# pmichels19/AdvancedGraphicsRayTracer

Measured on AMD Instinct MI355X. Metric: Mrays/s (primary+shadow) at 1080p, higher is better.
Workload: dtype f32

## Files before the change

advancedgraphicsraytracer_amd/__init__.py:

```python
import contextlib
import ctypes as C
import os

import numpy as np

PKG_DIR = os.path.dirname(os.path.abspath(__file__))
LIB_PATH = os.path.abspath(os.environ.get("RTAMD_LIB", os.path.join(PKG_DIR, "librtamd.so")))
DATA_DIR = os.path.join(PKG_DIR, "data")
HEADER = os.path.join(os.path.dirname(PKG_DIR), "include", "rt_amd.h")

ABI_VERSION = 4
RT_OK, RT_ERR_INVALID, RT_ERR_NO_DEVICE, RT_ERR_HIP, RT_ERR_IO, RT_ERR_UNSUPPORTED, RT_ERR_COMM = 0, -1, -2, -3, -4, -5, -6
RT_COMM_ID_BYTES = 128
MULTI_PIPELINED, MULTI_TIMING, MULTI_BALANCED = 1, 2, 4
SPHERE, PLANE, CUBE, QUAD, TRIANGLE = 0, 1, 2, 3, 4
DIFFUSE, MIRROR, DIELECTRIC, CHECKERBOARD, LIGHT, DSMIX, TEXTURE = 0, 1, 2, 3, 4, 5, 6
MODE_PATH = 0
MODE_WHITTED = 1
MODE_PACKET = 2
MODE_BVH_HEAT = 3
WALK_LANE, WALK_WAVE, WALK_AUTO = 0, 1, 2
WALK_CHECK_OFF, WALK_CHECK_COUNT, WALK_CHECK_VERIFY = 0, 1, 2
BVH_PLAIN, BVH_SBVH = 0, 1
DEFAULT_DEPTH = {MODE_PATH: 10, MODE_WHITTED: 20, MODE_PACKET: 10, MODE_BVH_HEAT: 1}
# ... 121 lines not shown
        "rt_bvh_visualize_host": ([vp, vp, vp, u32], C.c_int),
        "rt_scene_bvh_cost": ([vp, C.POINTER(BvhCost), vp], C.c_int),
        "rt_scene_update_triangles": ([vp, u32, u32, vp, vp], C.c_int),
        "rt_scene_update_triangles_host": ([vp, u32, u32, fp], C.c_int),
        "rt_scene_update_prims": ([vp, u32, u32, vp, vp, vp], C.c_int),
        "rt_scene_update_prims_host": ([vp, u32, u32, C.POINTER(Prim), fp], C.c_int),
        "rt_scene_transform_triangles": ([vp, C.POINTER(TriXform), u32, vp, vp], C.c_int),
        "rt_scene_update_triangles_async": ([vp, u32, u32, vp, vp, C.POINTER(C.c_uint64)], C.c_int),
        "rt_scene_update_prims_async": ([vp, u32, u32, vp, vp, vp, C.POINTER(C.c_uint64)], C.c_int),
        "rt_scene_transform_triangles_async": ([vp, C.POINTER(TriXform), u32, vp, vp, C.POINTER(C.c_uint64)], C.c_int),
        "rt_scene_update_sync": ([vp, C.POINTER(UpdateStatus)], C.c_int),
        "rt_scene_rebuild": ([vp, vp], C.c_int),
        "rt_scene_rebuild_stats": ([vp, C.POINTER(C.c_uint32)], C.c_int),
        "rt_scene_prepare_updates": ([vp, vp], C.c_int),
        "rt_scene_update_plan_info": ([vp, C.POINTER(C.c_uint32)], C.c_int),
        "rt_scene_copy_update_plan": ([vp, C.POINTER(u32), C.POINTER(u32), C.POINTER(u32)], C.c_int),
        "rt_bvh_refit_plan_host": ([vp, u32, C.POINTER(u32), u32, C.POINTER(C.POINTER(u32)), C.POINTER(C.POINTER(u32)),
                                    C.POINTER(C.POINTER(u32)), C.POINTER(u32)], C.c_int),
        "rt_scene_splice_triangles": ([vp, u32, u32, vp, u32, vp], C.c_int),
        "rt_scene_splice_triangles_host": ([vp, u32, u32, C.POINTER(Prim), u32], C.c_int),
        "rt_scene_splice_ranges": ([vp, C.POINTER(TriEdit), u32, vp, vp], C.c_int),
        "rt_scene_splice_ranges_host": ([vp, C.POINTER(TriEdit), u32, C.POINTER(Prim)], C.c_int),
        "rt_scene_compact_triangles": ([vp, vp, vp], C.c_int),
        "rt_scene_compact_triangles_host": ([vp, vp], C.c_int),
        "rt_scene_splice_prims": ([vp, C.POINTER(PrimEdit), u32, vp, vp, vp], C.c_int),
        "rt_scene_splice_prims_host": ([vp, C.POINTER(PrimEdit), u32, C.POINTER(Prim), fp], C.c_int),
        "rt_scene_compact_prims": ([vp, vp, vp], C.c_int),
        "rt_scene_compact_prims_host": ([vp, vp], C.c_int),
        "rt_scene_set_prim_materials": ([vp, u32, u32, vp, vp], C.c_int),
        "rt_scene_set_prim_materials_host": ([vp, u32, u32, C.POINTER(i32)], C.c_int),
        "rt_sbvh_build_host": ([C.POINTER(Prim), C.POINTER(C.c_float), u32, C.POINTER(vp), C.POINTER(C.POINTER(u32)),
                                C.POINTER(SceneInfo)], C.c_int),
        "rt_image_load": ([C.c_char_p, C.POINTER(C.POINTER(u32)), C.POINTER(u32), C.POINTER(u32)], C.c_int),
        "rt_scene_create": ([C.POINTER(SceneDesc), C.POINTER(vp)], C.c_int),
        "rt_scene_create_recipe": ([C.c_char_p, C.c_char_p, i32, C.POINTER(vp)], C.c_int),
        "rt_scene_create_recipe_ex": ([C.c_char_p, C.c_char_p, i32, i32, C.POINTER(vp)], C.c_int),
        "rt_scene_destroy": ([vp], C.c_int),
        "rt_scene_get_info": ([vp, C.POINTER(SceneInfo)], C.c_int),
        "rt_scene_set_camera_walk": ([vp, C.c_int], C.c_int),
        "rt_scene_copy_bvh": ([vp, vp, C.POINTER(u32)], C.c_int),
        "rt_intersect": ([vp, vp, vp, u32, vp], C.c_int),
        "rt_occluded": ([vp, vp, vp, u32, vp], C.c_int),
        "rt_intersect_host": ([vp, vp, vp, u32], C.c_int),
        "rt_occluded_host": ([vp, vp, vp, u32], C.c_int),
        "rt_intersect_packets": ([vp, vp, vp, u32, vp], C.c_int),
        "rt_intersect_packets_host": ([vp, vp, vp, u32], C.c_int),
        "rt_trace": ([vp, C.c_int, vp, vp, vp, u32, vp, vp, vp, u32, vp], C.c_int),
        "rt_trace_host": ([vp, C.c_int, vp, vp, vp, u32, vp, vp, vp, u32], C.c_int),
        "rt_comm_unique_id": ([vp], C.c_int),
        "rt_comm_create": ([vp, C.c_int, C.c_int, C.c_int, C.POINTER(vp)], C.c_int),
        "rt_comm_wrap": ([vp, C.c_int, C.POINTER(vp)], C.c_int),
        "rt_comm_info": ([vp, C.POINTER(C.c_int), C.POINTER(C.c_int)], C.c_int),
        "rt_comm_destroy": ([vp], C.c_int),
        "rt_render_frame_multi": ([vp, vp, C.POINTER(Camera), C.POINTER(FrameParams), vp, u32, vp], C.c_int),
        "rt_multi_flush": ([vp, vp, vp, vp], C.c_int),
        "rt_comm_timing": ([vp, C.POINTER(C.c_double), C.POINTER(C.c_double), C.POINTER(C.c_uint64)], C.c_int),
        "rt_comm_deal_info": ([vp, C.POINTER(C.c_int), C.POINTER(C.c_uint32), C.POINTER(C.c_uint32),
                               C.POINTER(C.c_uint64)], C.c_int),
        "rt_comm_deal_hash": ([vp, C.POINTER(C.c_uint64)], C.c_int),
        "rt_camera_default": ([u32, u32, C.POINTER(Camera)], C.c_int),
        "rt_renderer_create": ([vp, u32, u32, C.POINTER(vp)], C.c_int),
        "rt_renderer_destroy": ([vp], C.c_int),
        "rt_render_frame": ([vp, C.POINTER(Camera), C.POINTER(FrameParams), vp, vp], C.c_int),
        "rt_render_frame_host": ([vp, C.POINTER(Camera), C.POINTER(FrameParams), vp], C.c_int),
        "rt_render_gbuffer": ([vp, C.POINTER(Camera), C.POINTER(FrameParams), u32, u32, u32, u32, u32, C.POINTER(GBuffer), vp],
                              C.c_int),
        "rt_render_gbuffer_host": ([vp, C.POINTER(Camera), C.POINTER(FrameParams), u32, u32, u32, u32, u32, C.POINTER(GBuffer)],
                                   C.c_int),
        "rt_gbuffer_pixels": ([vp, C.POINTER(Camera), C.POINTER(FrameParams), u32, vp, u32, C.POINTER(GBuffer), vp], C.c_int),
        "rt_gbuffer_pixels_host": ([vp, C.POINTER(Camera), C.POINTER(FrameParams), u32, vp, u32, C.POINTER(GBuffer)], C.c_int),
        "rt_renderer_gbuffer_walk": ([vp, C.c_int, C.POINTER(C.c_int), C.POINTER(u32)], C.c_int),
        "rt_shard_capacity": ([u32, u32, u32, C.POINTER(u32)], C.c_int),
        "rt_render_shard": ([vp, C.POINTER(Camera), C.POINTER(FrameParams), u32, u32, vp, vp], C.c_int),
        "rt_assemble_shards": ([vp, vp, u32, vp, vp], C.c_int),
        "rt_tile_deal": ([u32, u32, C.POINTER(u32), u32, C.POINTER(u32), C.POINTER(u32)], C.c_int),
        "rt_render_shard_tiles": ([vp, C.POINTER(Camera), C.POINTER(FrameParams), C.POINTER(u32), u32, vp, vp], C.c_int),
        "rt_assemble_tiles": ([vp, vp, u32, C.POINTER(u32), C.POINTER(u32), u32, vp, vp], C.c_int),
        "rt_renderer_counters": ([vp, C.POINTER(Counters)], C.c_int),
        "rt_renderer_read_accumulator": ([vp, fp], C.c_int),
        "rt_renderer_overlap": ([vp, C.POINTER(C.c_int), fp], C.c_int),
        "rt_renderer_overlap_depth": ([vp, C.POINTER(C.c_int), fp], C.c_int),
        "rt_renderer_device_bytes": ([vp, C.POINTER(C.c_uint64), C.POINTER(C.c_uint32)], C.c_int),
        "rt_renderer_tile_costs": ([vp, C.POINTER(u32), u32, C.POINTER(u32)], C.c_int),
        "rt_renderer_tile_work": ([vp, C.POINTER(Camera), C.POINTER(FrameParams), C.POINTER(u32), u32, vp, vp], C.c_int),
        "rt_renderer_choices": ([vp, C.POINTER(C.c_int), C.POINTER(C.c_int), fp, fp], C.c_int),
        "rt_renderer_set_walk_check": ([vp, C.c_int], C.c_int),
        "rt_renderer_walk_stats": ([vp, C.POINTER(C.c_uint64)], C.c_int),
        "rt_renderer_stream": ([vp, C.POINTER(vp)], C.c_int),
        "rt_frame_kernel_name": ([vp, C.POINTER(FrameParams)], C.c_char_p),
        "rt_synchronize": ([vp], C.c_int),
    }
    for name, (args, res) in sigs.items():
        fn = getattr(L, name)
        fn.argtypes = args
        fn.restype = res
    if L.rt_abi_version() != ABI_VERSION:
        raise RTError(RT_ERR_INVALID, "librtamd.so ABI mismatch")
    _lib = L
    return L


def _check(rc):
    if rc != RT_OK:
        raise RTError(rc, lib().rt_last_error().decode(errors="replace"))
    return rc


def device_count():
    n = C.c_int(0)
    rc = lib().rt_device_count(C.byref(n))
    return n.value if rc == RT_OK else 0


def _fptr(a):
    return a.ctypes.data_as(C.POINTER(C.c_float))


def load_obj(path):
    return _take_mesh(lib().rt_obj_load, path)


def load_mesh(path):
    return _take_mesh(lib().rt_mesh_load, path)


def _take_mesh(fn, path):
    L = lib()
    vp, fp = C.POINTER(C.c_float)(), C.POINTER(C.c_int32)()
    nv, nt = C.c_uint32(), C.c_uint32()
    _check(fn(os.fsencode(path), C.byref(vp), C.byref(nv), C.byref(fp), C.byref(nt)))
    try:
        V = np.ctypeslib.as_array(vp, shape=(nv.value, 3)).copy() if nv.value else np.zeros((0, 3), np.float32)
        F = np.ctypeslib.as_array(fp, shape=(nt.value, 3)).copy() if nt.value else np.zeros((0, 3), np.int32)
    finally:
        L.rt_free(C.cast(vp, C.c_void_p))
        L.rt_free(C.cast(fp, C.c_void_p))
    return V, F


def save_mesh(path, verts, faces):
    V = np.ascontiguousarray(verts, np.float32)
    F = np.ascontiguousarray(faces, np.int32)
    _check(lib().rt_mesh_save(os.fsencode(path), _fptr(V), len(V), F.ctypes.data_as(C.POINTER(C.c_int32)), len(F)))


def mat4_translate(x, y, z):
    m = np.zeros(16, np.float32)
    _check(lib().rt_mat4_translate(x, y, z, _fptr(m)))
    return m


def mat4_scale(s):
    m = np.zeros(16, np.float32)
    _check(lib().rt_mat4_scale(s, _fptr(m)))
    return m


def mat4_rotate(axis, angle):
    m = np.zeros(16, np.float32)
    _check(lib().rt_mat4_rotate(axis, angle, _fptr(m)))
    return m


def mat4_mul(*ms):
    acc = np.ascontiguousarray(ms[0], np.float32).copy()
    for m in ms[1:]:
# ... 801 lines not shown
        if frame is None:
            self.frame += 1
        return out

    def render_shard_tiles(self, out, tiles, spp=1, depth=None, frame=None, reset=False, stream=None):
        torch = _torch()
        p = self.params(spp, depth, frame, reset)
        t = np.ascontiguousarray(tiles, np.uint32)
        s = stream if stream is not None else torch.cuda.current_stream(out.device).cuda_stream
        _check(self.L.rt_render_shard_tiles(self.h, C.byref(self.camera), C.byref(p), t.ctypes.data_as(C.POINTER(C.c_uint32)),
                                            len(t), C.c_void_p(out.data_ptr()), C.c_void_p(s)))
        if frame is None:
            self.frame += 1
        return out

    def assemble_tiles(self, gathered, stride_px, deal_tiles, deal_off, out, stream=None):
        torch = _torch()
        dt = np.ascontiguousarray(deal_tiles, np.uint32)
        do = np.ascontiguousarray(deal_off, np.uint32)
        s = stream if stream is not None else torch.cuda.current_stream(out.device).cuda_stream
        _check(self.L.rt_assemble_tiles(self.h, C.c_void_p(gathered.data_ptr()), stride_px,
                                        dt.ctypes.data_as(C.POINTER(C.c_uint32)), do.ctypes.data_as(C.POINTER(C.c_uint32)),
                                        len(do) - 1, C.c_void_p(out.data_ptr()), C.c_void_p(s)))
        return out

    def assemble(self, gathered, num_shards, out, stream=None):
        torch = _torch()
        s = stream if stream is not None else torch.cuda.current_stream(out.device).cuda_stream
        _check(self.L.rt_assemble_shards(self.h, C.c_void_p(gathered.data_ptr()), num_shards,
                                         C.c_void_p(out.data_ptr()), C.c_void_p(s)))
        return out

    def kernel_name(self, spp=1, depth=None):
        name = self.L.rt_frame_kernel_name(self.h, C.byref(self.params(spp, depth)))
        if name is None:
            raise RTError(-1, self.L.rt_last_error().decode())
        return name.decode()

    def counters(self):
        c = Counters()
        _check(self.L.rt_renderer_counters(self.h, C.byref(c)))
        return {n: int(getattr(c, n)) for n, _ in Counters._fields_}

    def overlap(self):
        st = C.c_int()
        ms = np.zeros(4, np.float32)
        _check(self.L.rt_renderer_overlap(self.h, C.byref(st), _fptr(ms)))
        return st.value, [round(float(x), 4) for x in ms]

    def overlap_depth(self):
        d = C.c_int()
        ms = np.zeros(8, np.float32)
        _check(self.L.rt_renderer_overlap_depth(self.h, C.byref(d), _fptr(ms)))
        return d.value, [round(float(x), 4) for x in ms]

    def device_bytes(self):
        b, n = C.c_uint64(), C.c_uint32()
        _check(self.L.rt_renderer_device_bytes(self.h, C.byref(b), C.byref(n)))
        return b.value, n.value

    def choices(self):
        w, sp = C.c_int(), C.c_int()
        wm, sm = np.zeros(4, np.float32), np.zeros(4, np.float32)
        _check(self.L.rt_renderer_choices(self.h, C.byref(w), C.byref(sp), _fptr(wm), _fptr(sm)))
        return {"walk": w.value, "split": sp.value, "walk_ms": [round(float(x), 4) for x in wm],
                "split_ms": [round(float(x), 4) for x in sm]}

    def set_walk_check(self, level):
        _check(self.L.rt_renderer_set_walk_check(self.h, level))

    def walk_stats(self):
        out = (C.c_uint64 * 4)()
        _check(self.L.rt_renderer_walk_stats(self.h, out))
        return {"walked": int(out[0]), "margin_boxes": int(out[1]), "retraced": int(out[2]), "verify_mismatch": int(out[3])}

    def tile_costs(self):
        n = C.c_uint32()
        _check(self.L.rt_renderer_tile_costs(self.h, None, 0, C.byref(n)))
        out = np.zeros(n.value, np.uint32)
        if n.value:
            _check(self.L.rt_renderer_tile_costs(self.h, out.ctypes.data_as(C.POINTER(C.c_uint32)), n.value, C.byref(n)))
        return out

    def tile_work(self, spp=1, depth=None, frame=None, pixels=False, stream=None):
        tx, ty = (self.width + 7) // 8, (self.height + 7) // 8
        work = np.zeros(tx * ty, np.uint32)
        p = self.params(spp, depth, frame)
        buf = None
        if pixels:
            torch = _torch()
            buf = torch.zeros(self.width * self.height * 8, dtype=torch.int32, device=f"cuda:{self.scene.device}")
        _check(self.L.rt_renderer_tile_work(self.h, C.byref(self.camera), C.byref(p),
                                            work.ctypes.data_as(C.POINTER(C.c_uint32)), len(work),
                                            None if buf is None else C.c_void_p(buf.data_ptr()),
                                            None if stream is None else C.c_void_p(stream)))
        if buf is None:
            return work
        return work, buf.view(-1, 8).cpu().numpy().view(np.uint32)

    def accumulator(self):
        acc = np.zeros((self.height * self.width, 4), np.float32)
        _check(self.L.rt_renderer_read_accumulator(self.h, _fptr(acc)))
        return acc
```

advancedgraphicsraytracer_amd/build.py:

```python
import os
import subprocess
import sys

PKG = os.path.dirname(os.path.abspath(__file__))
ROOT = os.path.dirname(PKG)
CSRC = os.path.join(PKG, "csrc")
LIB = os.path.join(PKG, "librtamd.so")
SOURCES = ["rt_host.cpp", "rt_device.hip", "rt_kern_core.hip", "rt_kern_ext.hip", "rt_multi.cpp", "rt_sbvh.cpp",
           "rt_refit.hip", "rt_build.hip", "rt_splice.hip", "rt_scene_pack.cpp", "rt_cost.hip", "rt_plan.hip", "rt_scene_edit.hip"]
HEADERS = ["rt_math.h", "rt_internal.h", "rt_libm.h", "rt_dev_types.h", "rt_variants.h", "rt_kernels.inc", "rt_refit.h", "rt_tune.h", "rt_sched.h",
           "rt_records.h", "rt_update.h", "rt_build.h", "rt_splice.h", "rt_cost.h", "rt_plan.h", "rt_scene.h", os.path.join("..", "..", "include", "rt_amd.h")]

HIPCC = os.environ.get("HIPCC", "/opt/rocm/bin/hipcc")
LIBS = ["-lz", "-ldl"]
FLAGS = ["--offload-arch=gfx950", "-O3", "-std=c++17", "-ffp-contract=off", "-fno-slp-vectorize", "-fPIC",
         "-shared",
         "-Wall", "-Wno-unused-function"]


def _source_hash():
    import hashlib
    h = hashlib.sha256()
    for f in [os.path.join(CSRC, x) for x in SOURCES + HEADERS] + [os.path.abspath(__file__)]:
        with open(f, "rb") as fh:
            h.update(os.path.basename(f).encode() + b"\0" + fh.read())
    h.update(" ".join(FLAGS + LIBS).encode())
    return h.hexdigest()


STAMP = LIB + ".srchash"


def _stale():
    if not os.path.exists(LIB) or not os.path.exists(STAMP):
        return True
    with open(STAMP) as f:
        return f.read().strip() != _source_hash()


def build(force=False, verbose=False):
    if not force and not _stale():
        return LIB
    objdir = os.path.join(PKG, "_obj")
    os.makedirs(objdir, exist_ok=True)
    compile_flags = [f for f in FLAGS if f != "-shared"]
    procs = []
    objs = []
    for f in SOURCES:
        obj = os.path.join(objdir, os.path.splitext(f)[0] + ".o")
        lang = ["-x", "hip"]
        cmd = [HIPCC] + compile_flags + lang + ["-c", os.path.join(CSRC, f), "-o", obj]
        if verbose:
            print(" ".join(cmd), file=sys.stderr)
        procs.append((f, subprocess.Popen(cmd, stdout=subprocess.PIPE, stderr=subprocess.PIPE, text=True)))
        objs.append(obj)
    for f, p in procs:
        out, err = p.communicate()
        if p.returncode != 0:
            raise RuntimeError(f"hipcc failed on {f} ({p.returncode}):\n{out}\n{err}")
    cmd = [HIPCC, "--offload-arch=gfx950", "-fPIC", "-shared", "--hip-link", "-o", LIB + ".tmp"] + objs + LIBS
    if verbose:
        print(" ".join(cmd), file=sys.stderr)
    r = subprocess.run(cmd, capture_output=True, text=True)
    if r.returncode != 0:
        raise RuntimeError(f"link failed ({r.returncode}):\n{r.stdout}\n{r.stderr}")
    os.replace(LIB + ".tmp", LIB)
    with open(STAMP, "w") as f:
        f.write(_source_hash() + "\n")
    return LIB


if __name__ == "__main__":
    print(build(force="--force" in sys.argv, verbose=True))
```

advancedgraphicsraytracer_amd/csrc/rt_dev_types.h:

```cpp
#pragma once
#include <hip/hip_runtime.h>

#include <cstdint>

#include "../../include/rt_amd.h"
#include "rt_variants.h"

namespace rt {

enum : uint32_t { T_TRI = 4, T_SPH = 0, T_PLANE = 1, T_CUBE = 2, T_QUAD = 3 };
enum : int { F_DIFFUSE = 0, F_SPECULAR = 1, F_MIX = 2, F_DIELECTRIC = 3, F_LIGHT = 4 };

struct DevMaterial {
    int kind, flag;
    float c0[3], c1[3];
    float ior, diffuse, specular;
    uint32_t tex_off, tex_w, tex_h;
    uint32_t pad_[2];
};
static_assert(sizeof(DevMaterial) == 64, "DevMaterial is read as four float4");

struct SceneView {
    const float4 *__restrict__ nodes;
    const float4 *__restrict__ prims;
    const float4 *__restrict__ shade;
    const DevMaterial *__restrict__ mats;
    const uint32_t *__restrict__ sky;
    const float4 *__restrict__ xprims;
    const uint32_t *__restrict__ tex;
    uint32_t sky_w, sky_h;
    int sky_const;
    float sky_rgb[3];
    float light_M[12];
    float light_c[3];
    float light_r, light_r2, light_invr;
    int light_mat;
    int light_quad;
    float light_qsize, light_area;
    float light_N[3];
    uint32_t root_word;
    int bounds_finite;
    uint32_t stack_entries;
    int wave_primary;
    int walk_check;
    float walk_margin;
    const float4 *__restrict__ quads;
    uint32_t quad_root;
    int quad_lanes;
    unsigned long long *walk_stats;
};

constexpr uint32_t kCounterSlots = 1024;

constexpr size_t kLdsLaunchMax = 65536;
constexpr size_t kWorkCounterBytes = 8u * 256u * sizeof(uint32_t);

struct FrameArgs {
    float cam_pos[3], cam_tl[3], cam_tr[3], cam_bl[3];
    float lens, rw, rh;
    uint32_t W, H, spp, depth, frame, reset;
    uint32_t shard, nshards, tiles_x, ntiles_local;
    const uint32_t *tile_map;
    uint32_t nchunks, nunits;
    float4 *samples;
    int packed_out;
    const uint32_t *order;
    uint32_t part_shift;
    uint32_t *tile_cost;
    float4 *acc;
    uint32_t *out;
    const uint32_t *fwd_src;
    uint32_t *fwd_dst;
    unsigned long long *counters;
};

struct FrameLaunch {
    FrameVariant v;
    dim3 grid;
    size_t lds_bytes;
    hipStream_t stream;
};

constexpr uint32_t kQueueSegs = 16;

struct PathArgs {
    uint32_t s0, batch_spp, npaths, level;
    uint32_t seg_cap;
    int dynamic;
    uint32_t *qhead;
    uint32_t drain_level, drain_below;
    float4 *state;
    float4 *rec;
    float4 *result;
    uint32_t *queue_in, *queue_out;
    uint32_t *qcount;
    float4 *sum;
    uint32_t *tile_cost;
};

struct TraceArgs {
    const rt_ray *rays;
    uint32_t *seeds;
    const uint8_t *flags;
    float *radiance;
    rt_hit *hits;
    unsigned long long *counts;
    uint32_t n, depth;
};

struct GBufferArgs {
    rt_ray *ray;
    rt_hit *hit;
    rt_gnormal *normal;
    rt_galbedo *albedo;
    uint32_t sample;
    uint32_t x0, y0, w, h;
    uint32_t tx0, ty0, ntx, ntiles;
    const uint32_t *pixels;
    uint32_t n;
};

struct Launchers {
    void (*frame)(const SceneView &S, const FrameArgs &F, const FrameLaunch &L);
    void (*work)(const SceneView &S, const FrameArgs &F, const FrameLaunch &L, uint32_t *tile_work, uint32_t *pixel_work);
    void (*intersect)(const SceneView &S, const rt_ray *rays, rt_hit *hits, uint32_t n, size_t lds, hipStream_t st);
    void (*occluded)(const SceneView &S, const rt_ray *rays, uint8_t *out, uint32_t n, size_t lds, hipStream_t st);
    void (*intersect_packet)(const SceneView &S, const rt_ray *rays, rt_hit *hits, uint32_t n, hipStream_t st);
    int (*pt_level)(const SceneView &S, const FrameArgs &F, const PathArgs &P, bool tex, size_t lds, uint32_t num_cus,
                    hipStream_t st);
    void (*pt_lanes)(const SceneView &S, const FrameArgs &F, const PathArgs &P, bool tex, size_t lds, uint32_t num_cus,
                     hipStream_t st);
    void (*pt_finish)(const FrameArgs &F, const PathArgs &P, bool last, hipStream_t st);
    void (*trace)(const SceneView &S, const TraceArgs &A, const FrameVariant &v, size_t lds, hipStream_t st);
    void (*gbuffer)(const SceneView &S, const FrameArgs &F, const GBufferArgs &G, const GBufferVariant &v, size_t lds,
                    hipStream_t st);
};
namespace kext {
const Launchers &launchers();
}
namespace kcore {
const Launchers &launchers();
void launch_heat(const SceneView &S, const FrameArgs &F, size_t lds, hipStream_t st);
void launch_visualize(const SceneView &S, const rt_ray *rays, uint32_t *counts, uint32_t n, size_t lds, hipStream_t st);
}
void launch_assemble(const uint32_t *gathered, uint32_t cap, uint32_t nshards, const uint32_t *where, uint32_t tiles_x,
                     uint32_t ntiles, uint32_t W, uint32_t H, uint32_t *out, hipStream_t st, uint32_t first = 0);

}
```

advancedgraphicsraytracer_amd/csrc/rt_device.hip:

```cpp
#include <hip/hip_runtime.h>

#include <algorithm>
#include <cmath>
#include <cstdlib>
#include <cstring>
#include <mutex>
#include <string>
#include <vector>

#include "rt_cost.h"
#include "rt_dev_types.h"
#include "rt_internal.h"
#include "rt_records.h"
#include "rt_refit.h"
#include "rt_scene.h"
#include "rt_sched.h"
#include "rt_tune.h"

using namespace rt;

constexpr int kPsMaxDepth = 8;
constexpr int kPtMaxSlots = 8;
inline int hw_queues() {
    const char *e = std::getenv("GPU_MAX_HW_QUEUES");
    const int v = e ? std::atoi(e) : 0;
    return v > 0 ? v : 4;
}

template <int N>
struct ResultRing {
    DevBuf buf[N];
    hipEvent_t fin[N] = {};
    bool fin_set[N] = {};

    int event(int b) {
        if (!fin[b]) HIP_TRY(hipEventCreateWithFlags(&fin[b], hipEventDisableTiming | hipEventReleaseToDevice));
        return RT_OK;
    }
    int ensure(int b, size_t bytes) {
        if (bytes <= buf[b].bytes) return RT_OK;
        fin_set[b] = false;
        return buf[b].grow(bytes, Wait::kDevice);
    }
    int drop_from(int k) {
        for (int b = k; b < N; ++b) {
            if (int rc = buf[b].release(); rc != RT_OK) return rc;
            fin_set[b] = false;
        }
        return RT_OK;
    }
    float4 *at(int b) const { return buf[b].template as<float4>(); }
};

struct rt_renderer {
    rt_scene *scene = nullptr;
    int device = 0;
    uint32_t W = 0, H = 0;
    float4 *d_acc = nullptr;
    unsigned long long *d_counters = nullptr;
    uint32_t *d_rgb = nullptr;
    uint64_t primary = 0, frames = 0;
    hipStream_t stream = nullptr;
    DevBuf d_order, d_cost;
    std::vector<uint32_t> host_cost;
    bool tail_bound = false;
    uint32_t order_n = 0;
    uint64_t order_key = 0;
    int order_state = 0;
    uint32_t order_split = 0;
    uint32_t order_parts = 2;
    TimedGroups walk_tg, split_tg, ps_tg;
    hipEvent_t tune_ev[4][16] = {};
    float walk_ms[4] = {}, split_ms[4] = {}, ps_ms[8] = {};
    int wave = -1;
    bool use_split = false;
    int ps_use = -1;
    uint64_t walk_key = 0;
    hipEvent_t stall_ev = nullptr;
    bool stall_armed = false;
    int walk_check = RT_WALK_CHECK_OFF;
    DevBuf d_pt[kPtMaxSlots];
    ResultRing<kPtMaxSlots + 1> pt_res;
    float4 *d_sum = nullptr;
    hipStream_t pt_stream[kPsMaxDepth] = {};
    int nstreams = 0;

    hipEvent_t pt_lv[kPsMaxDepth] = {};
    int pt_slot = 0, pt_parity = 0;
    uint32_t pt_nslots = 0;
    size_t pt_need = 0;
    bool pt_serial_last = false;
    uint64_t ps_last = 0;
    uint32_t ps_prev = 0;
    hipEvent_t ps_join = nullptr;
    hipEvent_t cost_ev = nullptr;
    ResultRing<kPsMaxDepth + 1> ps_res;
    uint32_t ps_count = 0;
    uint64_t gate_key = 0;
    int gate_state = 0;
    uint32_t gate_frames = 0;
    DevBuf d_samples;
    std::vector<uint32_t> map_host;
    int held_kind = 0;
    uint32_t held_shard = 0, held_nshards = 1;
    std::vector<uint32_t> held_list;
    uint64_t map_gen = 0, held_gen = 0;
    DevBuf d_work;
    DevBuf d_map;
    uint64_t map_hash = 0;
    DevBuf d_where;
    uint64_t where_hash = 0;
    TileGrid grid() const { return tile_grid(W, H); }
};

template <class R, class Fn>
void each_buffer(R &r, Fn f) {
    for (auto &b : r.d_pt) f(b);
    for (auto &b : r.pt_res.buf) f(b);
    for (auto &b : r.ps_res.buf) f(b);
    for (auto *b : {&r.d_samples, &r.d_order, &r.d_cost, &r.d_map, &r.d_work, &r.d_where}) f(*b);
}

namespace {

enum { kWalk, kSplit, kOverlap, kGate };

void free_scene(rt_scene *s) {
    if (!s) return;
    (void)hipSetDevice(s->device);
    (void)hipDeviceSynchronize();
    void *ptrs[] = {s->d_nodes, s->d_prims, s->d_shade, s->d_mats, s->d_sky, s->d_xprims, s->d_tex, s->d_scratch, s->d_quads, s->d_cost};
    for (void *p : ptrs)
        if (p) (void)hipFree(p);
    free_refit(s->refit);
    if (s->stream) (void)hipStreamDestroy(s->stream);
    delete s;
}

int ensure_device(int device) {
    int count = 0;
    if (hipGetDeviceCount(&count) != hipSuccess || count == 0)
        return fail(RT_ERR_NO_DEVICE, "no HIP device visible: the MI355X path has no CPU fallback");
    if (device < 0 || device >= count) return fail(RT_ERR_INVALID, "device index out of range");
    HIP_TRY(hipSetDevice(device));
    return RT_OK;
}

#ifndef RT_PT_QUADS_DEFAULT
#define RT_PT_QUADS_DEFAULT 0
#endif
int pack_options_from_env(PackOptions &o) {
    if (const char *e = std::getenv("RT_BVH")) {
        if (std::strcmp(e, "sbvh") != 0 && std::strcmp(e, "plain") != 0)
            return fail(RT_ERR_INVALID, std::string("RT_BVH must be 'plain' or 'sbvh', not '") + e + "'");
        o.bvh_kind = std::strcmp(e, "sbvh") == 0 ? RT_BVH_SBVH : RT_BVH_PLAIN;
    }
    if (const char *e = std::getenv("RT_WALK_MARGIN")) o.walk_margin = std::ldexp(1.0f, std::max(-40, std::min(-1, std::atoi(e))));
    if (const char *e = std::getenv("RT_WALK_STICKY")) o.sliver_lim = std::atoi(e) >= 0 ? 0.0 : std::ldexp(1.0, std::atoi(e));
    if (const char *e = std::getenv("RT_WALK_STICKY_SPHERES")) o.sticky_spheres = std::atoi(e) != 0;
    o.quads = RT_PT_QUADS_DEFAULT != 0;
    if (const char *e = std::getenv("RT_PT_QUADS")) o.quads = std::atoi(e) != 0;
    return RT_OK;
}

}

void rt::scene_tree_fields(rt_scene *s, uint32_t root_word, bool nested, bool bounds_finite) {
    s->stack_depth = pick_stack(s->bvh.depth);
    s->walk_fits = stack_admits_walk(s->stack_depth);
    s->nested = nested;
    SceneView &v = s->view;
    v.nodes = (const float4 *)s->d_nodes;
    v.prims = (const float4 *)s->d_prims;
    v.root_word = root_word;
    v.stack_entries = s->stack_depth;
    v.bounds_finite = bounds_finite ? 1 : 0;
    s->xcd_order = (size_t)s->bvh.nodes_used * 32u + (size_t)s->num_prims * 48u > (4u << 20);
    if (const char *e = std::getenv("RT_XCD_ORDER")) s->xcd_order = std::atoi(e) != 0;
    if (s->walk != RT_WALK_LANE && !(s->nested && s->walk_fits)) s->walk = RT_WALK_LANE;
}

namespace {

void scene_knobs_from_env(rt_scene *s) {
    if (const char *e = std::getenv("RT_PT_WAVEFRONT")) s->pt_wavefront = std::atoi(e) != 0;
    if (const char *e = std::getenv("RT_PT_DYNAMIC")) s->pt_dynamic = std::atoi(e) != 0;
    if (const char *e = std::getenv("RT_PT_LANES")) s->pt_lanes = std::atoi(e) != 0;
    if (const char *e = std::getenv("RT_PT_DRAIN_LEVEL")) s->pt_drain_level = (uint32_t)std::max(1, std::atoi(e));
    if (const char *e = std::getenv("RT_PT_DRAIN_ROUNDS")) s->pt_drain_rounds = std::max(0.0, std::atof(e));
    if (const char *e = std::getenv("RT_PT_DRAIN_SMALL")) s->pt_drain_small = (uint32_t)std::max(0, std::atoi(e));
    if (const char *e = std::getenv("RT_PT_SMALL_ROUNDS")) s->pt_small_rounds = std::max(0.0, std::atof(e));
    if (const char *e = std::getenv("RT_PT_SMALL_DRAIN_ROUNDS")) s->pt_small_drain_rounds = std::max(0.0, std::atof(e));
    if (const char *e = std::getenv("RT_TILE_ORDER")) s->tile_order = std::atoi(e) != 0;
    if (const char *e = std::getenv("RT_SPLIT_UNITS")) s->split_units = (uint32_t)std::max(0, std::atoi(e));
    if (const char *e = std::getenv("RT_FRAME_WAVES")) {
        const int w = std::atoi(e);
        s->frame_waves = w == 7 || w == 8 ? w : 0;
    }
    if (const char *e = std::getenv("RT_SPLIT_HEAVY")) s->heavy_split = std::max(-1, std::atoi(e));
    if (const char *e = std::getenv("RT_SPLIT_PARTS")) {
        const int k = std::atoi(e);
        s->split_parts = k >= 8 ? 8u : k >= 4 ? 4u : 2u;
    }
    if (const char *e = std::getenv("RT_PT_PIPELINE")) s->pt_pipeline = std::atoi(e) != 0;
    if (const char *e = std::getenv("RT_PT_SLOTS")) s->pt_slots = (uint32_t)std::max(2, std::min((int)kPtMaxSlots, std::atoi(e)));
    if (const char *e = std::getenv("RT_PS_PIPELINE")) s->ps_pipeline = std::max(-1, std::min(1, std::atoi(e)));
    if (const char *e = std::getenv("RT_PS_BUFFERS")) s->ps_buffers = (uint32_t)std::max(2, std::min(kPsMaxDepth + 1, std::atoi(e)));
    if (const char *e = std::getenv("RT_PS_DEPTH")) s->ps_depth = (uint32_t)std::max(2, std::min(kPsMaxDepth, std::atoi(e)));
    if (const char *e = std::getenv("RT_TUNE_DELAY_MS")) s->tune_delay_ms = (float)std::max(0.0, std::atof(e));
    if (const char *e = std::getenv("RT_PT_MEM_MB"))
        s->pt_mem_bytes = std::max<uint64_t>(1, std::strtoull(e, nullptr, 10)) << 20;
    const bool wave_ok = !s->has_cubes && s->nested && s->walk_fits;
    s->walk = wave_ok ? RT_WALK_AUTO : RT_WALK_LANE;
    if (const char *e = std::getenv("RT_WAVE_PRIMARY")) s->walk = std::atoi(e) != 0 && wave_ok ? RT_WALK_WAVE : RT_WALK_LANE;
}

int scene_create(const rt_scene_desc *d, rt_scene **out) {
    if (!d || !out) return fail(RT_ERR_INVALID, "rt_scene_create: empty or null description");
    *out = nullptr;
    PackOptions o;
    int rc = pack_options_from_env(o);
    if (rc != RT_OK) return rc;
    ScenePack p;
    if ((rc = pack_scene(d, o, p)) != RT_OK) return rc;
    if ((rc = ensure_device(d->device)) != RT_OK) return rc;

    rt_scene *s = new rt_scene();
    s->device = d->device;
    s->num_prims = d->num_prims;
    s->num_materials = d->num_materials;
    s->ext = p.ext;
    s->ext_fixed = p.ext_fixed;
    s->has_cubes = p.has_cubes;
    s->refit.boxes_finite = p.boxes_finite;
    s->quads = s->quad_lanes = p.has_quads;
    s->refit.sliver_lim = o.sliver_lim;
    s->refit.sticky_spheres = o.sticky_spheres;
    rc = upload(&s->d_nodes, p.nodes);
    if (rc == RT_OK) rc = upload(&s->d_prims, p.prims);
    if (rc == RT_OK) rc = upload(&s->d_shade, p.shade);
    if (rc == RT_OK) rc = upload(&s->d_mats, p.mats);
    if (rc == RT_OK) rc = upload(&s->d_sky, p.sky);
    if (rc == RT_OK) rc = upload(&s->d_xprims, p.xprims);
    if (rc == RT_OK) rc = upload(&s->d_tex, p.texels);
    if (rc == RT_OK && s->quads) rc = upload(&s->d_quads, p.quads);
    if (rc == RT_OK && hipStreamCreateWithFlags(&s->stream, hipStreamNonBlocking) != hipSuccess)
        rc = fail(RT_ERR_HIP, "hipStreamCreate failed");
    if (rc != RT_OK) { free_scene(s); return rc; }
    s->bvh = std::move(p.bvh);
    s->refit.pinfo = std::move(p.pinfo);
    s->refit.pbox = std::move(p.pbox);
    s->refit.pcen = std::move(p.pcen);

    SceneView &v = s->view;
    v = p.view;
    scene_tree_fields(s, p.view.root_word, p.nested, p.view.bounds_finite != 0);
    v.shade = (const float4 *)s->d_shade;
    v.mats = (const DevMaterial *)s->d_mats;
    v.sky = (const uint32_t *)s->d_sky;
    v.xprims = (const float4 *)s->d_xprims;
    v.tex = (const uint32_t *)s->d_tex;
    v.quads = s->quads ? (const float4 *)s->d_quads : nullptr;
    {
        hipDeviceProp_t prop;
        if (hipGetDeviceProperties(&prop, s->device) == hipSuccess && prop.multiProcessorCount > 0)
            s->num_cus = (uint32_t)prop.multiProcessorCount;
    }
    scene_knobs_from_env(s);
    *out = s;
    return RT_OK;
}

size_t stack_bytes(const rt_scene *s) { return (size_t)s->stack_depth * 256u * sizeof(uint32_t); }
size_t walk_bytes(const rt_scene *s, const SceneView &v) {
    return v.wave_primary ? (size_t)s->stack_depth * 4u * sizeof(uint32_t) : 0u;
}
// ... 154 lines not shown
        }
        if (!pipe) {
            const bool last = s0 + P.batch_spp >= F.spp;
            K.pt_finish(F, P, last, st);
        }
    }
    if (pipe) {
        for (int k = 0; k < (int)r->pt_nslots; ++k)
            if (used[k]) {
                HIP_TRY(hipEventRecord(r->pt_lv[k], r->pt_stream[k]));
                HIP_TRY(hipStreamWaitEvent(st, r->pt_lv[k], 0));
            }
        PathArgs P{};
        P.result = r->pt_res.at(par);
        P.sum = r->d_sum;
        P.s0 = 0;
        P.batch_spp = F.spp;
        K.pt_finish(F, P, true, st);
        HIP_TRY(hipEventRecord(r->pt_res.fin[par], st));
        r->pt_res.fin_set[par] = true;
    }
    HIP_TRY(hipGetLastError());
    return RT_OK;
}

int ensure_order(rt_renderer *r, uint64_t key, uint32_t n) {
    if (key == r->order_key && n == r->order_n) return RT_OK;
    r->order_key = key;
    r->order_state = 0;
    r->host_cost.clear();
    if (n != r->order_n) {
        HIP_TRY(hipDeviceSynchronize());
        r->order_n = 0;
        int rc = r->d_order.release();
        if (rc == RT_OK) rc = r->d_cost.release();
        if (rc == RT_OK) rc = r->d_order.grow(order_capacity(n) * sizeof(uint32_t));
        if (rc == RT_OK) rc = r->d_cost.grow(2u * (size_t)n * sizeof(uint32_t));
        if (rc != RT_OK) return rc;
        r->order_n = n;
    }
    return RT_OK;
}

struct FramePlan {
    uint64_t key = 0;
    bool gate_open = false, stalled = false;
    TimedFrame walk, split, ps;
    int cost_map = -1;
    bool walk_pending = false;
    uint32_t depth = 0, buf = 0, lane = 0;
};

int tile_order_step(rt_renderer *r, FrameArgs &F, bool split_ok, FramePlan &P) {
    const uint32_t n = F.ntiles_local;
    const int walk_phase = P.cost_map >= 0 ? P.cost_map : P.walk.decide ? 2 : P.walk_pending ? 3 : -1;
    if (P.key != r->order_key || n != r->order_n) {
        r->tail_bound = false;
        r->ps_tg.stop();
        r->ps_use = -1;
    }
    if (int rc = ensure_order(r, P.key, n); rc != RT_OK) return rc;
    uint32_t *const d_cost = r->d_cost.as<uint32_t>(), *const d_order = r->d_order.as<uint32_t>();
    int use = -1;
    if (walk_phase == 3) {
    } else if (r->order_state == 0) {
        if (walk_phase == 0 || walk_phase == 1) F.tile_cost = d_cost + (size_t)walk_phase * n;
        else if (walk_phase == 2) use = r->wave;
        else { F.tile_cost = d_cost; r->order_state = 1; }
    } else if (r->order_state == 1) {
        use = 0;
    }
    if (use >= 0) {
        HIP_TRY(hipDeviceSynchronize());
        std::vector<uint32_t> cost(n);
        HIP_TRY(hipMemcpy(cost.data(), d_cost + (size_t)use * n, n * sizeof(uint32_t), hipMemcpyDeviceToHost));
        r->host_cost = cost;
        r->tail_bound = tail_bound(cost, r->scene->num_cus, F.nchunks);
        const uint32_t k = split_count(n, r->scene->heavy_split, split_ok), parts = r->scene->split_parts;
        const TileWhere where{F.tiles_x, F.shard, F.nshards, F.tile_map ? r->map_host.data() : nullptr};
        const std::vector<uint32_t> ent = build_tile_order(cost, k, parts, r->scene->xcd_order && split_ok, where);
        HIP_TRY(hipMemcpy(d_order, ent.data(), ent.size() * sizeof(uint32_t), hipMemcpyHostToDevice));
        r->order_split = k;
        r->order_parts = parts;
        r->order_state = 2;
        r->use_split = k > 0 && r->scene->heavy_split > 0;
        r->split_tg.stop();
        if (k > 0 && r->scene->heavy_split < 0) {
            start_two_way(r->split_tg, false);
            if (int rc = ensure_events(r->tune_ev[kSplit], 8); rc != RT_OK) return rc;
        }
    }
    if (r->order_state == 2) {
        P.split = r->split_tg.next(P.gate_open, P.stalled);
        if (P.split.decide) {
            if (int rc = group_times(r->tune_ev[kSplit], 4, r->split_ms); rc != RT_OK) return rc;
            r->use_split = tuned_alternative(r->split_ms);
        }
        const bool split = P.split.group >= 0 ? alternative_group(P.split) : r->use_split;
        F.order = split ? d_order + n : d_order;
        F.nunits = order_units(F.ntiles_local, F.nchunks, split, r->order_split, r->order_parts);
        F.part_shift = part_shift(r->order_parts);
    }
    return RT_OK;
}

uint64_t param_key(const rt_renderer *r, const FrameArgs &F, const rt_camera *cam, const rt_frame_params *p) {
    uint64_t key = fnv1a(cam, sizeof(*cam));
    key = fnv1a(&p->width, sizeof(uint32_t) * 4, key);
    key = fnv1a(&p->mode, sizeof(uint32_t), key);
    key = fnv1a(&F.shard, sizeof(uint32_t) * 2, key);
    if (F.tile_map) key = fnv1a(&r->map_hash, sizeof(r->map_hash), key);
    return key;
}

int tune_gate(rt_renderer *r, uint64_t key, hipStream_t st, bool &open) {
    const float delay = r->scene->tune_delay_ms;
    if (key != r->gate_key) {
        r->gate_key = key;
        r->gate_state = 0;
    }
    if (delay <= 0.0f) r->gate_state = 3;
    if (r->gate_state == 3) { open = true; return RT_OK; }
    open = false;
    if (int rc = ensure_events(r->tune_ev[kGate], 2); rc != RT_OK) return rc;
    if (r->gate_state == 0) {
        HIP_TRY(hipEventRecord(r->tune_ev[kGate][0], st));
        r->gate_state = 1;
        r->gate_frames = 0;
    } else if (r->gate_state == 1) {
        if (++r->gate_frames % 8 == 0) {
            HIP_TRY(hipEventRecord(r->tune_ev[kGate][1], st));
            r->gate_state = 2;
        }
    } else if (hipEventQuery(r->tune_ev[kGate][1]) == hipSuccess) {
        float ms = 0.0f;
        HIP_TRY(hipEventElapsedTime(&ms, r->tune_ev[kGate][0], r->tune_ev[kGate][1]));
        r->gate_state = ms >= delay ? 3 : 1;
        open = r->gate_state == 3;
    }
    return RT_OK;
}

int frame_args(rt_renderer *r, const rt_camera *cam, const rt_frame_params *p, uint32_t shard, uint32_t nshards,
               const uint32_t *tiles, uint32_t ntiles_map, FrameArgs &F) {
    if (p->width != r->W || p->height != r->H)
        return fail(RT_ERR_INVALID, "frame size differs from the renderer's accumulator");
    if (p->spp == 0) return fail(RT_ERR_INVALID, "spp must be >= 1");
    if (p->mode > RT_MODE_BVH_HEAT) return fail(RT_ERR_INVALID, "unknown integrator mode");
    if (nshards == 0 || shard >= nshards) return fail(RT_ERR_INVALID, "bad shard index");
    HIP_TRY(hipSetDevice(r->scene->device));
    F = FrameArgs{};
    for (int i = 0; i < 3; ++i) {
        F.cam_pos[i] = cam->pos[i]; F.cam_tl[i] = cam->top_left[i];
        F.cam_tr[i] = cam->top_right[i]; F.cam_bl[i] = cam->bottom_left[i];
    }
    F.lens = cam->lens_radius;
    F.rw = 1.0f / (float)r->W;
    F.rh = 1.0f / (float)r->H;
    F.W = r->W; F.H = r->H; F.spp = p->spp; F.depth = p->depth; F.frame = p->frame; F.reset = p->reset ? 1 : 0;
    const TileGrid g = r->grid();
    F.shard = shard; F.nshards = nshards; F.tiles_x = g.tiles_x;
    F.ntiles_local = local_tiles(g.ntiles, shard, nshards);
    if (tiles) {
        int rc = set_tile_map(r, tiles, ntiles_map, g.ntiles);
        if (rc != RT_OK) return rc;
        F.ntiles_local = ntiles_map;
        F.tile_map = r->d_map.as<uint32_t>();
    }
    F.acc = r->d_acc;
    F.counters = r->d_counters;
    F.nchunks = 1;
    F.nunits = F.ntiles_local;
    return RT_OK;
}

int work_frame(rt_renderer *r, const rt_camera *cam, const rt_frame_params *p, uint32_t shard, uint32_t nshards,
               const uint32_t *tiles, uint32_t ntiles_map, std::vector<uint32_t> &work, uint32_t *pixel_work,
               hipStream_t st) {
    if (!r || !cam || !p) return fail(RT_ERR_INVALID, "work frame: null argument");
    if (p->mode != RT_MODE_PATH) return fail(RT_ERR_UNSUPPORTED, "work frame: RT_MODE_PATH frames only");
    if (p->depth > 32) return fail(RT_ERR_UNSUPPORTED, "Trace depth above 32");
    if (stack_bytes(r->scene) + kWorkCounterBytes > kLdsLaunchMax)
        return fail(RT_ERR_UNSUPPORTED, "work frame: this tree's stacks leave no LDS for the counters");
    FrameArgs F;
    int rc = frame_args(r, cam, p, shard, nshards, tiles, ntiles_map, F);
// ... 138 lines not shown
        P.batch_spp = F.spp;
        P.result = F.samples;
        launchers(s).pt_finish(F, P, true, st);
        HIP_TRY(hipGetLastError());
        if (o.depth > 0) {
            HIP_TRY(hipEventRecord(r->ps_res.fin[o.buf], st));
            r->ps_res.fin_set[o.buf] = true;
        }
    }
    if (o.ps.ev_after >= 0) HIP_TRY(hipEventRecord(r->tune_ev[kOverlap][o.ps.ev_after], st));
    if (r->walk_tg.running() || r->split_tg.active() || r->ps_tg.active()) {
        if (!r->stall_ev) HIP_TRY(hipEventCreateWithFlags(&r->stall_ev, hipEventDisableTiming));
        HIP_TRY(hipEventRecord(r->stall_ev, st));
        r->stall_armed = true;
    }
    return RT_OK;
}

int launch_render(rt_renderer *r, const rt_camera *cam, const rt_frame_params *p, uint32_t shard, uint32_t nshards,
                  uint32_t *out, int packed, void *stream, const uint32_t *tiles = nullptr, uint32_t ntiles_map = 0,
                  const uint32_t *fwd_src = nullptr, uint32_t *fwd_dst = nullptr) {
    if (!r || !cam || !p || !out) return fail(RT_ERR_INVALID, "rt_render: null argument");
    if ((fwd_src || fwd_dst) && (packed || !fwd_src || !fwd_dst)) return fail(RT_ERR_INVALID, "rt_render: bad forward");
    rt_scene *s = r->scene;
    FrameArgs F;
    if (int rc = frame_args(r, cam, p, shard, nshards, tiles, ntiles_map, F); rc != RT_OK) return rc;
    if (tiles) {
        if (r->held_kind != 3 || r->held_gen != r->map_gen) {
            r->held_list = r->map_host;
            r->held_gen = r->map_gen;
        }
        r->held_kind = 3;
    } else {
        r->held_kind = nshards == 1 ? 1 : 2;
        r->held_shard = shard;
        r->held_nshards = nshards;
    }
    F.packed_out = packed;
    F.out = out;
    F.fwd_src = fwd_src;
    F.fwd_dst = fwd_dst;
    if (F.ntiles_local == 0) return RT_OK;
    hipStream_t st = (hipStream_t)stream;
    if (int rc = after_updates(s, st); rc != RT_OK) return rc;
    if (p->mode == RT_MODE_BVH_HEAT) {
        F.depth = s->bvh.depth;
        kcore::launch_heat(s->view, F, stack_bytes(s), st);
        HIP_TRY(hipGetLastError());
        r->primary += frame_pixels(r, F) * p->spp;
        r->frames += 1;
        return RT_OK;
    }
    if (p->depth > 32) return fail(RT_ERR_UNSUPPORTED, "Trace depth above 32");
    const int mode = (int)p->mode;
    const bool wavefront = mode == RT_MODE_PATH && p->depth >= 2 && s->pt_wavefront;
    if (int rc = sample_split(r, p->spp, mode != RT_MODE_PACKET && !wavefront, F); rc != RT_OK) return rc;
    if (wavefront) {
        if (int rc = wavefront_frame(r, F, cam, p, st); rc != RT_OK) return rc;
        r->primary += frame_pixels(r, F) * p->spp;
        r->frames += 1;
        return RT_OK;
    }
    FrameLaunch L{{}, dim3((F.nunits + 3) / 4), stack_bytes(s), st};
    SceneView view = s->view;
    view.walk_stats = r->d_counters;
    view.walk_check = r->walk_check;
    FramePlan P;
    P.key = param_key(r, F, cam, p);
    if (int rc = tune_gate(r, P.key, st, P.gate_open); rc != RT_OK) return rc;
    P.stalled = r->stall_armed && hipEventQuery(r->stall_ev) == hipSuccess;
    r->stall_armed = false;
    const bool ps_kernel = primary_shadow(mode, p->depth);
    if (int rc = walk_step(r, ps_kernel && !s->ext, view, P); rc != RT_OK) return rc;
    if (s->tile_order) {
        if (int rc = tile_order_step(r, F, ps_kernel && F.nchunks <= 1, P); rc != RT_OK) return rc;
        L.grid = dim3((F.nunits + 3) / 4);
    }
    const uint64_t ps_bytes = (uint64_t)p->spp * F.ntiles_local * 64u * 16u;
    const bool ps_ok = s->ps_pipeline != 0 && ps_kernel && !r->split_tg.active() && !F.tile_cost && !P.walk_pending &&
                       ps_bytes <= (2ull << 30);
    if (int rc = overlap_step(r, F, L, ps_ok, ps_bytes, st, P); rc != RT_OK) return rc;
    if (L.stream != st)
        if (int rc = after_updates(s, L.stream); rc != RT_OK) return rc;
    L.lds_bytes = stack_bytes(s) + walk_bytes(s, view);
    L.v = frame_variant({mode, p->depth, !view.sky_const, s->frame_waves, F.nchunks, F.spp, F.nunits, s->num_cus,
                         P.depth > 0, view.wave_primary, view.walk_check});
    if (int rc = submit_frame(r, view, F, L, P, st); rc != RT_OK) return rc;
    r->primary += frame_pixels(r, F) * p->spp;
    r->frames += 1;
    return RT_OK;
}

template <class Launch>
int ray_call(rt_scene *s, const void *rays, void *out, uint32_t n, void *stream, const char *null_text, Launch launch) {
    if (!s || (n && (!rays || !out))) return fail(RT_ERR_INVALID, null_text);
    if (n == 0) return RT_OK;
    HIP_TRY(hipSetDevice(s->device));
    hipStream_t st = (hipStream_t)stream;
    if (int rc = after_updates(s, st); rc != RT_OK) return rc;
    launch(st);
    HIP_TRY(hipGetLastError());
    return RT_OK;
}

int gbuffer_arguments(const std::string &name, const void *r, const rt_camera *cam, const rt_frame_params *p, uint32_t sample,
                      const rt_gbuffer *out) {
    if (!r || !cam || !p || !out) return fail(RT_ERR_INVALID, name + ": null argument");
    if (!out->ray && !out->hit && !out->normal && !out->albedo) return fail(RT_ERR_INVALID, name + ": no plane asked for");
    if (sample >= std::max(1u, p->spp)) return fail(RT_ERR_INVALID, name + ": sample outside the frame's samples per pixel");
    return RT_OK;
}
int gbuffer_rectangle(const std::string &name, const rt_frame_params *p, uint32_t x0, uint32_t y0, uint32_t w, uint32_t h) {
    if (!w || !h) return fail(RT_ERR_INVALID, name + ": empty rectangle");
    if (x0 >= p->width || w > p->width - x0 || y0 >= p->height || h > p->height - y0)
        return fail(RT_ERR_INVALID, name + ": the rectangle leaves the frame");
    return RT_OK;
}
int gbuffer_device() {
    static const bool have = [] {
        int count = 0;
        return hipGetDeviceCount(&count) == hipSuccess && count > 0;
    }();
    return have ? RT_OK : fail(RT_ERR_NO_DEVICE, "no HIP device visible: the MI355X path has no CPU fallback");
}
SceneView gbuffer_view(const rt_renderer *r, bool pixels, size_t &lds) {
    const rt_scene *s = r->scene;
    SceneView view = s->view;
    view.wave_primary = gbuffer_wave_walk({pixels, s->walk, r->wave, s->ext, s->has_cubes, s->nested, s->walk_fits}) ? 1 : 0;
    view.walk_check = RT_WALK_CHECK_OFF;
    view.walk_stats = nullptr;
    lds = stack_bytes(s) + walk_bytes(s, view);
    return view;
}
int gbuffer_launch(rt_renderer *r, const rt_camera *cam, const rt_frame_params *p, GBufferArgs &G, bool pixels, hipStream_t st) {
    if (int rc = gbuffer_device(); rc != RT_OK) return rc;
    rt_frame_params q = *p;
    q.spp = std::max(1u, p->spp);
    q.mode = RT_MODE_PATH;
    FrameArgs F;
    if (int rc = frame_args(r, cam, &q, 0, 1, nullptr, 0, F); rc != RT_OK) return rc;
    F.acc = nullptr;
    F.counters = nullptr;
    if (pixels && G.n == 0) return RT_OK;
    rt_scene *s = r->scene;
    if (int rc = after_updates(s, st); rc != RT_OK) return rc;
    size_t lds = 0;
    const SceneView view = gbuffer_view(r, pixels, lds);
    launchers(s).gbuffer(view, F, G, gbuffer_variant(pixels, !view.sky_const), lds, st);
    HIP_TRY(hipGetLastError());
    return RT_OK;
}
GBufferArgs gbuffer_planes(const rt_gbuffer *out, uint32_t sample) {
    GBufferArgs G{};
    G.ray = out->ray; G.hit = out->hit; G.normal = out->normal; G.albedo = out->albedo;
    G.sample = sample;
    return G;
}
template <class Run>
int gbuffer_staged(rt_renderer *r, const rt_frame_params *p, const uint32_t *list, size_t count, const rt_gbuffer *out, Run run) {
    if (int rc = gbuffer_device(); rc != RT_OK) return rc;
    if (p->width != r->W || p->height != r->H) return fail(RT_ERR_INVALID, "frame size differs from the renderer's accumulator");
    if (count == 0) return RT_OK;
    rt_scene *s = r->scene;
    HIP_TRY(hipSetDevice(s->device));
    auto up = [](size_t b) { return (b + 255) & ~(size_t)255; };
    void *const host[4] = {out->ray, out->hit, out->normal, out->albedo};
// ... 255 lines not shown
             : kind == CALL_VISUALIZE ? rt_bvh_visualize(s, d_rays, (uint32_t *)d_out, n, s->stream)
                                    : rt_intersect(s, d_rays, (rt_hit *)d_out, n, s->stream);
    if (rc != RT_OK) return rc;
    HIP_TRY(hipMemcpyAsync(out, d_out, out_elem * n, hipMemcpyDeviceToHost, s->stream));
    HIP_TRY(hipStreamSynchronize(s->stream));
    return RT_OK;
}

int rt_intersect_host(rt_scene *s, const rt_ray *rays, rt_hit *hits, uint32_t n) {
    return staged_call(s, rays, hits, sizeof(rt_hit), n, CALL_INTERSECT);
}
int rt_occluded_host(rt_scene *s, const rt_ray *rays, uint8_t *out, uint32_t n) {
    return staged_call(s, rays, out, 1, n, CALL_OCCLUDED);
}
int rt_intersect_packets_host(rt_scene *s, const rt_ray *rays, rt_hit *hits, uint32_t n) {
    return staged_call(s, rays, hits, sizeof(rt_hit), n, CALL_PACKETS);
}

int rt_bvh_visualize(rt_scene *s, const rt_ray *rays, uint32_t *counts, uint32_t n, void *stream) {
    return ray_call(s, rays, counts, n, stream, "rt_bvh_visualize: null argument",
                    [&](hipStream_t st) { kcore::launch_visualize(s->view, rays, counts, n, stack_bytes(s), st); });
}
int rt_bvh_visualize_host(rt_scene *s, const rt_ray *rays, uint32_t *counts, uint32_t n) {
    return staged_call(s, rays, counts, 2 * sizeof(uint32_t), n, CALL_VISUALIZE);
}

int rt_scene_bvh_cost(rt_scene *s, rt_bvh_cost *out, void *stream) {
    if (!s || !out) return fail(RT_ERR_INVALID, "rt_scene_bvh_cost: null argument");
    if (int frc = fold_updates(s); frc != RT_OK) return frc;
    if (!s->view.bounds_finite) return fail(RT_ERR_UNSUPPORTED, "rt_scene_bvh_cost: a node bound is NaN or infinite");
    HIP_TRY(hipSetDevice(s->device));
    rt_bvh_cost c{};
    const int rc = device_bvh_cost(s->d_nodes, s->bvh.nodes_used, &s->d_cost, (hipStream_t)stream, &c);
    if (rc == RT_OK) *out = c;
    return rc;
}

int rt_renderer_create(rt_scene *s, uint32_t W, uint32_t H, rt_renderer **out) {
    if (!s || !out || !W || !H) return fail(RT_ERR_INVALID, "rt_renderer_create: bad argument");
    if ((uint64_t)W * H >= (1ull << 31)) return fail(RT_ERR_UNSUPPORTED, "frame too large");
    HIP_TRY(hipSetDevice(s->device));
    rt_renderer *r = new rt_renderer();
    r->scene = s;
    r->device = s->device;
    r->W = W; r->H = H;
    start_two_way(r->walk_tg, true);
    hipError_t e = hipStreamCreateWithFlags(&r->stream, hipStreamNonBlocking);
    if (e == hipSuccess) e = hipMalloc(&r->d_acc, sizeof(float4) * (size_t)W * H);
    if (e == hipSuccess) e = hipMemsetAsync(r->d_acc, 0, sizeof(float4) * (size_t)W * H, r->stream);
    if (e == hipSuccess) e = hipMalloc(&r->d_counters, kCounterSlots * 8 * sizeof(unsigned long long));
    if (e == hipSuccess) e = hipMemsetAsync(r->d_counters, 0, kCounterSlots * 8 * sizeof(unsigned long long), r->stream);
    if (e == hipSuccess) e = hipStreamSynchronize(r->stream);
    if (e != hipSuccess) {
        if (r->d_acc) (void)hipFree(r->d_acc);
        if (r->d_counters) (void)hipFree(r->d_counters);
        if (r->stream) (void)hipStreamDestroy(r->stream);
        delete r;
        return fail(RT_ERR_HIP, std::string("rt_renderer_create: ") + hipGetErrorString(e));
    }
    *out = r;
    return RT_OK;
}

int rt_renderer_destroy(rt_renderer *r) {
    if (!r) return RT_OK;
    (void)hipSetDevice(r->device);
    (void)hipDeviceSynchronize();
    (void)hipFree(r->d_acc);
    (void)hipFree(r->d_counters);
    if (r->d_rgb) (void)hipFree(r->d_rgb);
    if (r->d_sum) (void)hipFree(r->d_sum);
    each_buffer(*r, [](DevBuf &b) { (void)b.release(); });
    for (int k = 0; k < kPsMaxDepth; ++k) {
        if (r->pt_stream[k]) (void)hipStreamDestroy(r->pt_stream[k]);
        if (r->pt_lv[k]) (void)hipEventDestroy(r->pt_lv[k]);
    }
    for (auto &row : r->tune_ev)
        for (auto &e : row)
            if (e) (void)hipEventDestroy(e);
    for (hipEvent_t e : r->pt_res.fin)
        if (e) (void)hipEventDestroy(e);
    for (hipEvent_t e : r->ps_res.fin)
        if (e) (void)hipEventDestroy(e);
    for (hipEvent_t e : {r->ps_join, r->cost_ev, r->stall_ev})
        if (e) (void)hipEventDestroy(e);
    (void)hipStreamDestroy(r->stream);
    delete r;
    return RT_OK;
}

int rt_render_frame(rt_renderer *r, const rt_camera *cam, const rt_frame_params *p, uint32_t *rgb8, void *stream) {
    return launch_render(r, cam, p, 0, 1, rgb8, 0, stream);
}

int rt_render_frame_host(rt_renderer *r, const rt_camera *cam, const rt_frame_params *p, uint32_t *rgb8) {
    if (!r || !rgb8) return fail(RT_ERR_INVALID, "rt_render_frame_host: null argument");
    HIP_TRY(hipSetDevice(r->scene->device));
    if (!r->d_rgb) HIP_TRY(hipMalloc(&r->d_rgb, sizeof(uint32_t) * (size_t)r->W * r->H));
    int rc = launch_render(r, cam, p, 0, 1, r->d_rgb, 0, r->stream);
    if (rc != RT_OK) return rc;
    HIP_TRY(hipMemcpyAsync(rgb8, r->d_rgb, sizeof(uint32_t) * (size_t)r->W * r->H, hipMemcpyDeviceToHost, r->stream));
    HIP_TRY(hipStreamSynchronize(r->stream));
    return RT_OK;
}

int rt_render_gbuffer(rt_renderer *r, const rt_camera *cam, const rt_frame_params *p, uint32_t sample, uint32_t x0, uint32_t y0,
                      uint32_t w, uint32_t h, const rt_gbuffer *out, void *stream) {
    const char *name = "rt_render_gbuffer";
    if (int rc = gbuffer_arguments(name, r, cam, p, sample, out); rc != RT_OK) return rc;
    if (int rc = gbuffer_rectangle(name, p, x0, y0, w, h); rc != RT_OK) return rc;
    GBufferArgs G = gbuffer_planes(out, sample);
    G.x0 = x0; G.y0 = y0; G.w = w; G.h = h;
    G.tx0 = x0 / 8u; G.ty0 = y0 / 8u;
    G.ntx = (x0 + w + 7u) / 8u - G.tx0;
    G.ntiles = G.ntx * ((y0 + h + 7u) / 8u - G.ty0);
    return gbuffer_launch(r, cam, p, G, false, (hipStream_t)stream);
}

int rt_render_gbuffer_host(rt_renderer *r, const rt_camera *cam, const rt_frame_params *p, uint32_t sample, uint32_t x0,
                           uint32_t y0, uint32_t w, uint32_t h, const rt_gbuffer *out) {
    const char *name = "rt_render_gbuffer_host";
    if (int rc = gbuffer_arguments(name, r, cam, p, sample, out); rc != RT_OK) return rc;
    if (int rc = gbuffer_rectangle(name, p, x0, y0, w, h); rc != RT_OK) return rc;
    return gbuffer_staged(r, p, nullptr, (size_t)w * h, out, [&](const uint32_t *, const rt_gbuffer *dev, hipStream_t st) {
        return rt_render_gbuffer(r, cam, p, sample, x0, y0, w, h, dev, st);
    });
}

int rt_gbuffer_pixels(rt_renderer *r, const rt_camera *cam, const rt_frame_params *p, uint32_t sample, const uint32_t *pixels,
                      uint32_t n, const rt_gbuffer *out, void *stream) {
    const char *name = "rt_gbuffer_pixels";
    if (int rc = gbuffer_arguments(name, r, cam, p, sample, out); rc != RT_OK) return rc;
    if (n && !pixels) return fail(RT_ERR_INVALID, std::string(name) + ": null pixel list");
    GBufferArgs G = gbuffer_planes(out, sample);
    G.pixels = pixels;
    G.n = n;
    return gbuffer_launch(r, cam, p, G, true, (hipStream_t)stream);
}

int rt_gbuffer_pixels_host(rt_renderer *r, const rt_camera *cam, const rt_frame_params *p, uint32_t sample,
                           const uint32_t *pixels, uint32_t n, const rt_gbuffer *out) {
    const char *name = "rt_gbuffer_pixels_host";
    if (int rc = gbuffer_arguments(name, r, cam, p, sample, out); rc != RT_OK) return rc;
    if (n && !pixels) return fail(RT_ERR_INVALID, std::string(name) + ": null pixel list");
    for (uint32_t i = 0; i < n; ++i)
        if (pixels[i] >= (uint64_t)p->width * p->height)
            return fail(RT_ERR_INVALID, std::string(name) + ": pixel " + std::to_string(i) + " lies outside the frame");
    return gbuffer_staged(r, p, pixels, n, out, [&](const uint32_t *list, const rt_gbuffer *dev, hipStream_t st) {
        return rt_gbuffer_pixels(r, cam, p, sample, list, n, dev, st);
    });
}

int rt_renderer_gbuffer_walk(const rt_renderer *r, int pixels, int *wave_walk, uint32_t *lds_bytes) {
    if (!r || !wave_walk) return fail(RT_ERR_INVALID, "rt_renderer_gbuffer_walk: null argument");
    size_t lds = 0;
    *wave_walk = gbuffer_view(r, pixels != 0, lds).wave_primary;
    if (lds_bytes) *lds_bytes = (uint32_t)lds;
    return RT_OK;
}

int rt_shard_capacity(uint32_t W, uint32_t H, uint32_t nshards, uint32_t *pixels) {
    if (!pixels || !nshards || !W || !H) return fail(RT_ERR_INVALID, "rt_shard_capacity: bad argument");
    *pixels = local_tiles(tile_grid(W, H).ntiles, 0, nshards) * 64u;
    return RT_OK;
}

int rt_render_shard(rt_renderer *r, const rt_camera *cam, const rt_frame_params *p, uint32_t shard, uint32_t nshards,
// ... 79 lines not shown
    std::vector<unsigned long long> c((size_t)kCounterSlots * 8);
    HIP_TRY(hipMemcpy(c.data(), r->d_counters, c.size() * sizeof(unsigned long long), hipMemcpyDeviceToHost));
    for (int i = 0; i < 4; ++i) out[i] = 0;
    for (uint32_t k = 0; k < kCounterSlots; ++k) {
        out[0] += c[(size_t)k * 8 + 4];
        out[1] += c[(size_t)k * 8 + 2];
        out[2] += c[(size_t)k * 8 + 3];
        out[3] += c[(size_t)k * 8 + 5];
    }
    return RT_OK;
}

int rt_renderer_overlap(const rt_renderer *r, int *state, float ms[4]) {
    if (!r || !state) return fail(RT_ERR_INVALID, "rt_renderer_overlap: null argument");
    int depth = 0;
    float all[8];
    rt_renderer_overlap_depth(r, &depth, all);
    *state = depth < 0 ? -1 : (depth > 1 ? 1 : 0);
    if (ms) {
        const int n = r->ps_tg.groups == 8 ? 8 : 4;
        const int g[4] = {0, 1, n - 2, n - 1};
        for (int k = 0; k < 4; ++k) ms[k] = all[g[k]];
    }
    return RT_OK;
}

int rt_renderer_choices(const rt_renderer *r, int *walk, int *split, float walk_ms[4], float split_ms[4]) {
    if (!r || !walk || !split) return fail(RT_ERR_INVALID, "rt_renderer_choices: null argument");
    const rt_scene *s = r->scene;
    const bool split_set = r->order_state == 2 && !r->split_tg.active();
    *walk = s->walk == RT_WALK_WAVE ? 1 : s->walk == RT_WALK_LANE ? 0 : r->wave;
    *split = split_set ? (r->use_split ? 1 : 0) : -1;
    for (int g = 0; g < 4; ++g) {
        if (walk_ms) walk_ms[g] = (r->wave >= 0 && s->walk == RT_WALK_AUTO) ? r->walk_ms[g] : 0.0f;
        if (split_ms) split_ms[g] = split_set ? r->split_ms[g] : 0.0f;
    }
    return RT_OK;
}

int rt_renderer_overlap_depth(const rt_renderer *r, int *depth, float ms[8]) {
    if (!r || !depth) return fail(RT_ERR_INVALID, "rt_renderer_overlap_depth: null argument");
    const int32_t mode = r->scene->ps_pipeline;
    const bool decided = mode < 0 && r->ps_use >= 0;
    if (mode == 0) *depth = 1;
    else if (mode == 1) *depth = (int)r->scene->ps_depth;
    else *depth = decided ? (r->ps_use ? r->ps_use : 1) : -1;
    if (ms)
        for (int g = 0; g < 8; ++g) ms[g] = (decided && g < r->ps_tg.groups) ? r->ps_ms[g] : 0.0f;
    return RT_OK;
}

int rt_renderer_device_bytes(const rt_renderer *r, uint64_t *bytes, uint32_t *ps_buffers) {
    if (!r || !bytes) return fail(RT_ERR_INVALID, "rt_renderer_device_bytes: null argument");
    const uint64_t pix = (uint64_t)r->W * r->H;
    uint64_t b = 16u * pix + kCounterSlots * 8u * sizeof(unsigned long long);
    if (r->d_rgb) b += 4u * pix;
    if (r->d_sum) b += sum_bytes(r);
    each_buffer(*r, [&](const DevBuf &x) { b += x.bytes; });
    uint32_t nps = 0;
    for (const DevBuf &x : r->ps_res.buf) nps += x.p != nullptr;
    *bytes = b;
    if (ps_buffers) *ps_buffers = nps;
    return RT_OK;
}

int rt_renderer_tile_work(rt_renderer *r, const rt_camera *cam, const rt_frame_params *p, uint32_t *work, uint32_t n,
                          uint32_t *pixel_work_dev, void *stream) {
    if (!r || !cam || !p || (n && !work)) return fail(RT_ERR_INVALID, "rt_renderer_tile_work: null argument");
    if (n < r->grid().ntiles) return fail(RT_ERR_INVALID, "rt_renderer_tile_work: room for every tile needed");
    std::vector<uint32_t> w;
    int rc = work_frame(r, cam, p, 0, 1, nullptr, 0, w, pixel_work_dev, (hipStream_t)stream);
    if (rc != RT_OK) return rc;
    std::memcpy(work, w.data(), sizeof(uint32_t) * w.size());
    return RT_OK;
}

int rt_renderer_tile_costs(const rt_renderer *r, uint32_t *costs, uint32_t n, uint32_t *n_out) {
    if (!r || !n_out || (n && !costs)) return fail(RT_ERR_INVALID, "rt_renderer_tile_costs: null argument");
    *n_out = (uint32_t)r->host_cost.size();
    if (n && !r->host_cost.empty()) std::memcpy(costs, r->host_cost.data(), sizeof(uint32_t) * std::min<size_t>(n, r->host_cost.size()));
    return RT_OK;
}

int rt_renderer_read_accumulator(rt_renderer *r, float *host) {
    if (!r || !host) return fail(RT_ERR_INVALID, "null argument");
    HIP_TRY(hipSetDevice(r->scene->device));
    HIP_TRY(hipDeviceSynchronize());
    HIP_TRY(hipMemcpy(host, r->d_acc, sizeof(float4) * (size_t)r->W * r->H, hipMemcpyDeviceToHost));
    return RT_OK;
}

const char *rt_frame_kernel_name(const rt_renderer *r, const rt_frame_params *p) {
    if (r && p && p->mode == RT_MODE_BVH_HEAT) return "k_render_heat";
    if (!r || !p || p->mode > RT_MODE_PACKET || p->depth > 32) {
        fail(RT_ERR_INVALID, "rt_frame_kernel_name: bad argument");
        return nullptr;
    }
    const rt_scene *s = r->scene;
    if (p->mode == RT_MODE_PATH && p->depth >= 2 && s->pt_wavefront) return "k_pt_level";
    return frame_variant_name(kernel_class((int)p->mode, p->depth, !s->view.sky_const));
}

int rt_renderer_stream(rt_renderer *r, void **stream) {
    if (!r || !stream) return fail(RT_ERR_INVALID, "null argument");
    *stream = (void *)r->stream;
    return RT_OK;
}

int rt_synchronize(rt_renderer *r) {
    if (!r) return fail(RT_ERR_INVALID, "null argument");
    HIP_TRY(hipSetDevice(r->scene->device));
    HIP_TRY(hipDeviceSynchronize());
    return RT_OK;
}

}
```

advancedgraphicsraytracer_amd/csrc/rt_kernels.inc:

```
#include <hip/hip_runtime.h>

#include <algorithm>
#include <cstdint>
#include <map>
#include <mutex>
#include <tuple>
#include <type_traits>

#include "rt_dev_types.h"
#include "rt_libm.h"
#include "rt_math.h"

#ifndef RT_KNS
#error "define RT_KNS (kcore / kext) and RT_EXT (0 / 1) before including rt_kernels.inc"
#endif

namespace rt {
namespace RT_KNS {

constexpr bool kExt = RT_EXT != 0;

#ifdef RT_FRAME_PHASES
constexpr uint32_t kFramePhaseWaves = 65536;
__device__ unsigned long long rt_frame_phase_buf[kFramePhaseWaves * 8u];
// ... 794 lines not shown
        if (last) { rnd_u(seed); rnd_u(seed); }
        else out = make_ray(I, diffuse_dir(N, seed), 1e34f);
        return false;
    }
}

__device__ __forceinline__ f3 texture_color(const SceneView &S, const DevMaterial &m, const DRay &in) {
    const uint32_t u = f2u_wrap((float)m.tex_w * in.u), v = f2u_wrap((float)m.tex_h * in.v);
    const uint32_t p = S.tex[m.tex_off + (u & (m.tex_w - 1)) + (v & (m.tex_h - 1)) * m.tex_w];
    return mk((float)((p >> 16) & 255), (float)((p >> 8) & 255), (float)(p & 255)) * (1.0f / 255.0f);
}

__device__ __forceinline__ f3 mat_color(const SceneView &S, const DevMaterial &m, const DRay &in, f3 I) {
    if (kExt && m.kind == RT_TEXTURE) return texture_color(S, m, in);
    if (m.kind == RT_DIELECTRIC) {
        f3 c = mk(1, 1, 1);
        if (in.inside) { c.x = exp_f(-m.c0[0] * in.t); c.y = exp_f(-m.c0[1] * in.t); c.z = exp_f(-m.c0[2] * in.t); }
        return c;
    }
    if (m.kind == RT_CHECKERBOARD) {
        bool ex = abs(((int)floorf(I.x)) % 2) == 0;
        bool ez = abs(((int)floorf(I.z)) % 2) == 0;
        return ex == ez ? mk(m.c0[0], m.c0[1], m.c0[2]) : mk(m.c1[0], m.c1[1], m.c1[2]);
    }
    return mk(m.c0[0], m.c0[1], m.c0[2]);
}

__device__ __forceinline__ f3 light_point(const SceneView &S, uint32_t &seed) {
    if (kExt && S.light_quad) {
        const float a = S.light_qsize * (rnd_f(seed) - 1.0f);
        const float b = S.light_qsize * (rnd_f(seed) - 1.0f);
        return tpos(S.light_M, mk(a, b, 0.0f));
    }
    f3 pt = mk(1, 1, 1);
    while (dot(pt, pt) > 1) {
        float x = rnd_sym(seed);
        float y = rnd_sym(seed);
        float z = rnd_sym(seed);
        pt = mk(x, y, z);
    }
    return tpos(S.light_M, normalize(pt) * S.light_r);
}

template <class TR, bool EARLY = false>
__device__ __forceinline__ f3 nee(const SceneView &S, const TR &T, f3 I, f3 N, f3 BRDF, uint32_t &seed,
                                  uint32_t &nshadow) {
    f3 Il = light_point(S, seed);
    float area = S.light_area;
    f3 lc0 = mk(0, 0, 0);
    if constexpr (EARLY) {
        if constexpr (!kExt) {
            const DevMaterial &lm = S.mats[S.light_mat];
            lc0 = mk(lm.c0[0], lm.c0[1], lm.c0[2]);
            asm volatile("" : "+v"(lc0.x), "+v"(lc0.y), "+v"(lc0.z));
        }
        asm volatile("" : "+v"(area));
    }
    f3 L = Il - I;
    float dist = length(L);
    L = L / dist;
    f3 Nl = (kExt && S.light_quad) ? mk(S.light_N[0], S.light_N[1], S.light_N[2])
                                   : (Il - mk(S.light_c[0], S.light_c[1], S.light_c[2])) * S.light_invr;
    if (dot(Nl, L) > 0) Nl = -Nl;
    float dotNL = dot(N, L), dotNlL = dot(Nl, -L);
    f3 Ld = mk(0, 0, 0);
    frame_phase(3);
    if (dotNL > 0 && dotNlL > 0) {
        DRay sh = make_ray(I, L, dist - 2.0f * kEPS);
        ++nshadow;
        if (!occluded(S, T, sh)) {
            float solid = (dotNlL * area) / (dist * dist);
            float lightPDF = 1.0f / solid;
            const DevMaterial &lm = S.mats[S.light_mat];
            const f3 lc = !kExt ? (EARLY ? lc0 : mk(lm.c0[0], lm.c0[1], lm.c0[2])) : mat_color(S, lm, sh, sh.O + sh.t * sh.D);
            Ld = (lc * BRDF) * (dotNL / lightPDF);
        }
    }
    frame_phase(4);
    return Ld;
}

template <int MAXD, bool TEX_SKY, class TR, int CAMWAVE = 0, bool WHOLE = false>
__device__ f3 trace_path(const SceneView &S, const TR &T, DRay ray, int depth, uint32_t &seed,
                         uint32_t &nshadow, uint32_t &nbounce, bool lastSpec = true) {
    f3 lv_mul[MAXD], lv_add[MAXD];
    float lv_c[MAXD];
    bool lv_diff[MAXD];
    int levels = 0;
    f3 term = mk(0, 0, 0);
    for (int d = depth; d > 0 && levels < MAXD; --d) {
        if (d != depth) ++nbounce;
        if constexpr (CAMWAVE) {
            if (d == depth) closest_hit_primary<CAMWAVE == 2>(S, T, ray);
            else closest_hit(S, T, ray);
        } else {
            closest_hit(S, T, ray);
        }
        frame_phase(2);
        if (ray.obj == -1) { term = sky_color<TEX_SKY>(S, ray.D); break; }
        f3 I = ray.O + ray.t * ray.D;
        f3 N;
        DevMaterial m_whole;
        if constexpr (WHOLE) m_whole = hit_surface_whole(S, ray, I, N);
        const DevMaterial &m = WHOLE ? m_whole : hit_surface(S, ray, I, N);
        if (m.flag == F_LIGHT) { term = lastSpec ? mk(m.c0[0], m.c0[1], m.c0[2]) : mk(0, 0, 0); break; }
        const bool last = MAXD == 1 || d == 1;
        DRay out;
        bool spec = scatter(m, ray, I, N, out, seed, last);
        f3 albedo = mat_color(S, m, ray, I);
        if (m.flag == F_DIFFUSE || (m.flag == F_MIX && !spec)) {
            f3 BRDF = albedo * kINVPI;
            lv_add[levels] = nee<TR, WHOLE>(S, T, I, N, BRDF, seed, nshadow);
            lv_mul[levels] = BRDF;
            lv_c[levels] = last ? 0.0f : dot(N, out.D);
            lv_diff[levels] = true;
        } else {
            lv_mul[levels] = albedo;
            lv_add[levels] = mk(0, 0, 0);
            lv_c[levels] = 0.0f;
            lv_diff[levels] = false;
        }
        ++levels;
        if (last) break;
        ray = out;
        lastSpec = spec;
    }
    f3 r = term;
    for (int k = levels - 1; k >= 0; --k)
        r = lv_diff[k] ? lv_mul[k] * ((r * lv_c[k]) / kINV2PI) + lv_add[k] : lv_mul[k] * r;
    return r;
}

template <int MAXD, bool TEX_SKY, class TR>
__device__ f3 shade_packet(const SceneView &S, const TR &T, DRay ray, int depth, uint32_t &seed,
                           uint32_t &nshadow, uint32_t &nbounce) {
    if (ray.obj == -1) return sky_color<TEX_SKY>(S, ray.D);
    f3 I = ray.O + ray.t * ray.D;
    f3 N;
    const DevMaterial &m = hit_surface(S, ray, I, N);
    const bool last = depth == 0;
    DRay out;
    bool spec = scatter(m, ray, I, N, out, seed, last);
    f3 albedo = mat_color(S, m, ray, I);
    if (m.flag == F_LIGHT) return albedo;
    const bool diffuse = m.flag == F_DIFFUSE || m.flag == F_MIX;
    const int passes = (m.flag == F_MIX && spec) ? 2 : 1;
    const f3 BRDF = albedo * kINVPI;
    f3 Ld = mk(0, 0, 0), Li = mk(0, 0, 0);
    for (int p = 0; p < passes; ++p) {
        if (diffuse && p == passes - 1) Ld = nee(S, T, I, N, BRDF, seed, nshadow);
        nbounce += last ? 0u : 1u;
        Li = trace_path<MAXD, TEX_SKY>(S, T, out, depth, seed, nshadow, nbounce, spec);
    }
    if (!diffuse) return albedo * Li;
    f3 Ei = (Li * (last ? 0.0f : dot(N, out.D))) / kINV2PI;
    return BRDF * Ei + Ld;
}

__device__ __forceinline__ void color_modifier(const SceneView &S, const DevMaterial &m, const DRay &in, f3 I, f3 N, f3 &c, float &c3,
                                               f3 &T) {
    c3 = 0.0f;
    T = mk(0, 0, 0);
    switch (m.kind) {
    case RT_LIGHT:
        c = mk(fmaxf(0.0f, fminf(m.c0[0], 1.0f)), fmaxf(0.0f, fminf(m.c0[1], 1.0f)), fmaxf(0.0f, fminf(m.c0[2], 1.0f)));
        return;
    case RT_CHECKERBOARD:
    case RT_TEXTURE:
        c = mat_color(S, m, in, I);
        c3 = m.diffuse;
        return;
    case RT_DSMIX:
        c = mk(m.c0[0], m.c0[1], m.c0[2]);
        c3 = m.diffuse;
        return;
    case RT_DIELECTRIC: {
        float n1 = 1, n2 = m.ior, n12 = n1 / n2;
        float cosi = dot(N, in.D);
        c = mk(1, 1, 1);
        if (in.inside) {
            c = mk(exp_f(-m.c0[0] * in.t), exp_f(-m.c0[1] * in.t), exp_f(-m.c0[2] * in.t));
            n12 = 1 / n12;
        }
        float k = 1 - (n12 * n12) * (1 - (cosi * cosi));
        if (k < 0) { c3 = -1.0f; return; }
        if (!in.inside) {
            float sini = length(cross(N, in.D));
            float sq = n12 * sini;
            float cost = sqrtf(1 - sq * sq);
            c3 = fresnel(n1, n2, cost, -cosi);
        }
        T = normalize(n12 * in.D - (n12 * cosi + sqrtf(k)) * N);
        return;
    }
    default:
        c = mk(m.c0[0], m.c0[1], m.c0[2]);
        return;
    }
}

template <class TR>
__device__ __forceinline__ f3 direct_illumination(const SceneView &S, const TR &T, f3 I, f3 N,
                                                  uint32_t &seed, uint32_t &nshadow) {
    f3 result = mk(0, 0, 0);
    const f3 ldir = mk(0.0f, -1.0f, 0.0f), lcol = mk(24.0f, 24.0f, 22.0f);
    for (int i = 0; i < 4; ++i) {
        f3 L = light_point(S, seed) - I;
        float dist = length(L);
        L = L / dist;
        float dotDN = dot(L, N);
        if (dotDN < 0 || dot(ldir, L) > 0) continue;
        DRay sh = make_ray(I, L, dist - (2 * kEPS));
        ++nshadow;
        if (occluded(S, T, sh)) continue;
        result = result + (dotDN / (dist * dist)) * lcol;
    }
    return result / 4.0f;
}

constexpr int kWHITTED_MAX = 32;
struct WFrame {
    f3 col, res, I, T;
    float w, ft;
    int flags;
};

template <bool TEX_SKY, class TR>
__device__ f3 trace_whitted(const SceneView &S, const TR &T, DRay ray, int depth, uint32_t &seed,
                            uint32_t &nshadow, uint32_t &nbounce) {
    WFrame st[kWHITTED_MAX];
    int sp = 0;
    bool primary = true;
    for (;;) {
        f3 ret = mk(0, 0, 0);
        if (depth - sp > 0) {
            if (!primary) ++nbounce;
            primary = false;
            closest_hit(S, T, ray);
            if (ray.obj == -1) {
                ret = sky_color<TEX_SKY>(S, ray.D);
            } else {
                f3 I = ray.O + ray.t * ray.D;
                f3 N;
                const DevMaterial &m = hit_surface(S, ray, I, N);
                f3 col, Tdir;
                float c3;
                color_modifier(S, m, ray, I, N, col, c3, Tdir);
                f3 res = mk(0, 0, 0);
                WFrame f;
                f.col = col; f.w = 1.0f; f.ft = 0.0f; f.flags = 0;
                bool push = false, child_inside = false;
                f3 childD = mk(0, 0, 0);
                if (m.flag == F_LIGHT) {
                    res = res + mk(24.0f, 24.0f, 22.0f);
                } else if (m.flag == F_DIFFUSE) {
                    res = res + direct_illumination(S, T, I, N, seed, nshadow);
                } else if (m.flag == F_SPECULAR) {
                    push = true; childD = normalize(reflect(ray.D, N));
                } else if (m.flag == F_MIX) {
                    res = res + c3 * direct_illumination(S, T, I, N, seed, nshadow);
                    push = true; childD = normalize(reflect(ray.D, N));
                    f.w = 1.0f - c3; f.flags = 1;
                } else if (m.flag == F_DIELECTRIC) {
                    if (c3 < 0) {
                        push = true; childD = normalize(reflect(ray.D, N)); child_inside = true;
                    } else {
                        float Fr = c3, Ft = 1 - Fr;
                        if (Fr > kFLT_EPSILON) {
                            push = true; childD = normalize(reflect(ray.D, N));
                            f.w = Fr; f.flags = 1;
                            if (Ft > kFLT_EPSILON) {
                                f.flags |= 2 | (ray.inside ? 0 : 4);
                                f.ft = Ft; f.I = I; f.T = Tdir;
                            }
                        } else if (Ft > kFLT_EPSILON) {
                            push = true; childD = Tdir; child_inside = !ray.inside;
                            f.w = Ft; f.flags = 1;
                        }
                    }
                }
                if (push) {
                    f.res = res;
                    st[sp++] = f;
                    ray = make_ray(I, childD, 1e34f);
                    ray.inside = child_inside ? 1 : 0;
                    continue;
                }
                ret = col * res;
            }
        }
        bool descend = false;
        while (sp > 0) {
            WFrame &f = st[sp - 1];
            f.res = f.res + ((f.flags & 1) ? f.w * ret : ret);
            if (f.flags & 2) {
                ray = make_ray(f.I, f.T, 1e34f);
                ray.inside = (f.flags & 4) ? 1 : 0;
                f.w = f.ft;
                f.flags &= ~2;
                descend = true;
                break;
            }
            ret = f.col * f.res;
            --sp;
        }
        if (!descend) return ret;
    }
}

__device__ __forceinline__ DRay primary_ray(const FrameArgs &F, uint32_t x, uint32_t y, uint32_t &seed) {
    float u = (float)x * F.rw + rnd_f(seed) * F.rw;
    float v = (float)y * F.rh + rnd_f(seed) * F.rh;
    f3 p;
    for (;;) {
        float px = rnd_sym(seed);
        float py = rnd_sym(seed);
        p = mk(px, py, 0);
        if (!(dot(p, p) >= 1)) break;
    }
    f3 rd = F.lens * p;
    f3 offset = mk(u * rd.x, v * rd.y, 0);
    f3 pos = mk(F.cam_pos[0], F.cam_pos[1], F.cam_pos[2]);
    f3 tl = mk(F.cam_tl[0], F.cam_tl[1], F.cam_tl[2]);
    f3 tr = mk(F.cam_tr[0], F.cam_tr[1], F.cam_tr[2]);
    f3 bl = mk(F.cam_bl[0], F.cam_bl[1], F.cam_bl[2]);
    f3 P = tl + u * (tr - tl) + v * (bl - tl);
    return make_ray(pos + offset, normalize(P - pos - offset), 1e34f);
}

__device__ __forceinline__ uint32_t wave_sum(uint32_t v) {
    for (int o = 32; o > 0; o >>= 1) v += __shfl_xor(v, o, 64);
    return v;
}

__device__ __forceinline__ uint32_t pack_rgb8(float4 a) {
    uint32_t r = f2u_wrap(255.0f * smin(1.0f, a.x));
    uint32_t g = f2u_wrap(255.0f * smin(1.0f, a.y));
    uint32_t b = f2u_wrap(255.0f * smin(1.0f, a.z));
    return (r << 16) + (g << 8) + b;
}

__device__ __forceinline__ uint32_t global_tile(const FrameArgs &F, uint32_t local_tile) {
    return F.tile_map ? F.tile_map[local_tile] : local_tile * F.nshards + F.shard;
}

template <bool BINARY = false>
__device__ __forceinline__ void count_rays(const FrameArgs &F, uint32_t wave, uint32_t lane, uint32_t nshadow,
                                           uint32_t nbounce) {
    if constexpr (BINARY) {
        nshadow = (uint32_t)__popcll(__ballot(nshadow != 0u));
        nbounce = 0u;
    } else {
        nshadow = wave_sum(nshadow);
        nbounce = wave_sum(nbounce);
    }
    if (lane == 0) {
        unsigned long long *c = F.counters + (size_t)(wave % kCounterSlots) * 8u;
        if (nshadow) atomicAdd(&c[0], (unsigned long long)nshadow);
        if (nbounce) atomicAdd(&c[1], (unsigned long long)nbounce);
    }
}

enum : int { M_PATH = RT_MODE_PATH, M_WHITTED = RT_MODE_WHITTED, M_PACKET = RT_MODE_PACKET };

template <int MODE, int MAXD, bool TEX_SKY, class TR, bool WALKCHECK = false, bool ONE = false, bool DRY = false>
__device__ __forceinline__ void render_tile(const SceneView &S, const FrameArgs &F, const TR &T,
                                            uint32_t unit, uint32_t lane) {
    frame_phase(0);
    const uint32_t slot = F.nchunks <= 1 ? unit : unit / F.nchunks;
    const uint32_t entry = F.order ? F.order[slot] : slot;
    const uint32_t local_tile = entry & 0x0fffffffu;
    const bool part_tile = (entry >> 31) != 0u;
    const uint32_t chunk = F.nchunks <= 1 ? 0u : unit % F.nchunks;
    const uint64_t t_start = F.tile_cost ? __builtin_amdgcn_s_memtime() : 0;
    const uint32_t s_begin = chunk * F.spp / F.nchunks, s_end = (chunk + 1u) * F.spp / F.nchunks;
    const uint32_t tile = global_tile(F, local_tile);
    const uint32_t x = (tile % F.tiles_x) * 8u + (lane & 7u), y = (tile / F.tiles_x) * 8u + (lane >> 3);
    const bool on = x < F.W && y < F.H && (!part_tile || (lane >> F.part_shift) == ((entry >> 28) & 7u));
    const uint32_t px = x + y * F.W;
    constexpr bool kEarlyAcc = ONE && !DRY;
    float4 acc_in = make_float4(0, 0, 0, 0);
    if constexpr (kEarlyAcc) {
        uintptr_t fa = (uintptr_t)&F;
        asm volatile("" : "+s"(fa));
        const auto *Fh = (const __attribute__((address_space(4))) FrameArgs *)fa;
        const uint32_t reset = Fh->reset;
        const float4 *const samples = Fh->samples, *const acc = Fh->acc;
        if (on & (reset == 0u) & (samples == nullptr)) {
            typedef float f32x4 __attribute__((ext_vector_type(4)));
            const f32x4 v = *(const __attribute__((address_space(1))) f32x4 *)(uintptr_t)(acc + px);
            acc_in = make_float4(v.x, v.y, v.z, v.w);
        }
    }
    constexpr int kCamWave = (MODE == M_PATH && MAXD == 1 && TR::kStride == 256) ? (WALKCHECK ? 2 : 1) : 0;
    uint32_t nshadow = 0, nbounce = 0;
    f3 sum = mk(0, 0, 0);
    if (MODE == M_PACKET) {
        for (uint32_t s = 0; s < F.spp; ++s) {
            uint32_t seed = init_seed(px + F.W * F.H * (s + F.spp * F.frame));
            DRay ray = on ? primary_ray(F, x, y, seed) : make_ray(mk(0, 0, 0), mk(0, 0, 1), 1e34f);
            packet_closest_hit(S, ray, on);
            if (on) sum = sum + shade_packet<MAXD, TEX_SKY>(S, T, ray, (int)F.depth, seed, nshadow, nbounce);
        }
    } else if (ONE && on) {
        uint32_t seed = init_seed(px + F.W * F.H * (s_begin + F.spp * F.frame));
        DRay ray = primary_ray(F, x, y, seed);
        frame_phase(1);
        sum = trace_path<MAXD, TEX_SKY, TR, kCamWave, true>(S, T, ray, (int)F.depth, seed, nshadow, nbounce);
        if (F.samples) {
            F.samples[((size_t)s_begin * F.ntiles_local + local_tile) * 64u + lane] = make_float4(sum.x, sum.y, sum.z, 0.0f);
        }
    } else if (on) {
        for (uint32_t s = s_begin; s < s_end; ++s) {
            uint32_t seed = init_seed(px + F.W * F.H * (s + F.spp * F.frame));
            DRay ray = primary_ray(F, x, y, seed);
            f3 v;
            if constexpr (MODE == M_WHITTED) v = trace_whitted<TEX_SKY>(S, T, ray, (int)F.depth, seed, nshadow, nbounce);
            else v = trace_path<MAXD, TEX_SKY, TR, kCamWave>(S, T, ray, (int)F.depth, seed, nshadow, nbounce);
            if (F.samples) F.samples[((size_t)s * F.ntiles_local + local_tile) * 64u + lane] = make_float4(v.x, v.y, v.z, 0.0f);
            else sum = sum + v;
        }
    }
    if constexpr (DRY) return;
    if (on && !F.samples) {
        f3 res = (1.0f / (float)F.spp) * sum;
        float4 a;
        if constexpr (kEarlyAcc) a = acc_in;
        else a = F.reset ? make_float4(0, 0, 0, 0) : F.acc[px];
        a.w += 1;
        const float w = a.w, inv = 1.0f / w;
        a = make_float4(a.x + inv * (res.x - a.x), a.y + inv * (res.y - a.y), a.z + inv * (res.z - a.z),
                        a.w + inv * (w - a.w));
        F.acc[px] = a;
        const uint32_t rgb = pack_rgb8(a);
        if (F.packed_out) F.out[local_tile * 64u + lane] = rgb;
        else {
            if (F.fwd_dst) F.fwd_dst[px] = F.fwd_src[px];
            F.out[px] = rgb;
        }
    }
    count_rays<MODE == M_PATH && MAXD == 1 && ONE>(F, unit, lane, nshadow, nbounce);
    if (F.tile_cost && lane == 0) F.tile_cost[local_tile] = (uint32_t)(__builtin_amdgcn_s_memtime() - t_start);
    frame_phase(5);
}

#ifndef RT_RENDER_WAVES_PER_SIMD
#define RT_RENDER_WAVES_PER_SIMD 1
#endif
template <int MODE, int MAXD, bool TEX_SKY>
__global__ __launch_bounds__(256, RT_RENDER_WAVES_PER_SIMD) void k_render(SceneView S, FrameArgs F) {
    extern __shared__ uint32_t lds_stack[];
    const uint32_t tid = threadIdx.x;
    const uint32_t unit = blockIdx.x * 4u + (tid >> 6);
    if (unit >= F.nunits) return;
    Trav<256> T{S.nodes, lds_stack + tid, S.prims};
    render_tile<MODE, MAXD, TEX_SKY>(S, F, T, unit, tid & 63u);
}
struct FrameKernArgs { SceneView S; FrameArgs F; };
template <bool TEX_SKY>
__global__ __launch_bounds__(256, 8) void k_render_w8(SceneView, FrameArgs) {
    const auto *ka = (const FrameKernArgs *)__builtin_amdgcn_kernarg_segment_ptr();
    const SceneView &S = ka->S;
    const FrameArgs &F = ka->F;
    extern __shared__ uint32_t lds_stack[];
    const uint32_t tid = threadIdx.x;
    const uint32_t unit = blockIdx.x * 4u + (tid >> 6);
    if (unit >= F.nunits) return;
    Trav<256> T{S.nodes, lds_stack + tid, S.prims};
    render_tile<M_PATH, 1, TEX_SKY, Trav<256>, false, true>(S, F, T, unit, tid & 63u);
}
template <bool TEX_SKY>
__global__ __launch_bounds__(256, RT_RENDER_WAVES_PER_SIMD) void k_render_walkcheck(SceneView S, FrameArgs F) {
    extern __shared__ uint32_t lds_stack[];
    const uint32_t tid = threadIdx.x;
    const uint32_t unit = blockIdx.x * 4u + (tid >> 6);
    if (unit >= F.nunits) return;
    Trav<256> T{S.nodes, lds_stack + tid, S.prims};
    render_tile<M_PATH, 1, TEX_SKY, Trav<256>, true>(S, F, T, unit, tid & 63u);
}

template <int MAXD, bool TEX_SKY>
__global__ __launch_bounds__(256) void k_render_work(SceneView S, FrameArgs F, uint32_t *__restrict__ tile_work,
                                                     uint32_t *__restrict__ pixel_work, int with_dist) {
    extern __shared__ uint32_t lds_stack[];
    const uint32_t tid = threadIdx.x, lane = tid & 63u;
    const uint32_t unit = blockIdx.x * 4u + (tid >> 6);
    if (unit >= F.nunits) return;
    float *dist = with_dist ? reinterpret_cast<float *>(lds_stack + (size_t)S.stack_entries * 256u) + tid : nullptr;
    uint32_t *work = lds_stack + (size_t)S.stack_entries * (with_dist ? 512u : 256u) + tid;
    for (int k = 0; k < 8; ++k) work[k * 256] = 0u;
    Trav<256, true> T{S.nodes, lds_stack + tid, S.prims, work, dist};
    render_tile<M_PATH, MAXD, TEX_SKY, Trav<256, true>, false, false, true>(S, F, T, unit, lane);
    const uint32_t c0 = work[0], c1 = work[256], c2 = work[512], c3 = work[768];
    const uint32_t tot = wave_sum(c0 + c1 + c2 + c3);
    if (lane == 0) atomicAdd(&tile_work[unit], tot);
    if (pixel_work) {
        const uint32_t tile = global_tile(F, unit);
        const uint32_t x = (tile % F.tiles_x) * 8u + (lane & 7u), y = (tile / F.tiles_x) * 8u + (lane >> 3);
        if (x < F.W && y < F.H) {
            uint4 *q = reinterpret_cast<uint4 *>(pixel_work) + 2u * (x + (size_t)y * F.W);
            q[0] = make_uint4(c0, c1, c2, c3);
            q[1] = make_uint4(work[1024], work[1280], 0u, 0u);
        }
    }
}

__global__ __launch_bounds__(256) void k_intersect(SceneView S, const rt_ray *__restrict__ rays, rt_hit *__restrict__ hits,
                                                   uint32_t n) {
    extern __shared__ uint32_t lds_stack[];
    const uint32_t i = blockIdx.x * 256u + threadIdx.x;
    if (i >= n) return;
    rt_ray q = rays[i];
    DRay r = make_ray(mk(q.ox, q.oy, q.oz), mk(q.dx, q.dy, q.dz), q.tmax);
    Trav<256> T{S.nodes, lds_stack + threadIdx.x, S.prims};
    closest_hit(S, T, r);
    finish_uv(S, r);
    rt_hit h;
    h.t = r.t; h.obj = r.obj; h.u = r.u; h.v = r.v;
    hits[i] = h;
}

__global__ __launch_bounds__(256) void k_intersect_packet(SceneView S, const rt_ray *__restrict__ rays,
                                                          rt_hit *__restrict__ hits, uint32_t n) {
    const uint32_t i = blockIdx.x * 256u + threadIdx.x;
    if ((i & ~63u) >= n) return;
    const bool active = i < n;
    DRay r = make_ray(mk(0, 0, 0), mk(0, 0, 1), 1e34f);
    if (active) {
        rt_ray q = rays[i];
        r = make_ray(mk(q.ox, q.oy, q.oz), mk(q.dx, q.dy, q.dz), q.tmax);
    }
    packet_closest_hit(S, r, active);
    if (!active) return;
    finish_uv(S, r);
    rt_hit h;
    h.t = r.t; h.obj = r.obj; h.u = r.u; h.v = r.v;
    hits[i] = h;
}

__global__ __launch_bounds__(256) void k_occluded(SceneView S, const rt_ray *__restrict__ rays, uint8_t *__restrict__ out,
                                                  uint32_t n) {
    extern __shared__ uint32_t lds_stack[];
    const uint32_t i = blockIdx.x * 256u + threadIdx.x;
    if (i >= n) return;
    rt_ray q = rays[i];
    DRay r = make_ray(mk(q.ox, q.oy, q.oz), mk(q.dx, q.dy, q.dz), q.tmax);
    Trav<256> T{S.nodes, lds_stack + threadIdx.x, S.prims};
    out[i] = occluded(S, T, r) ? 1 : 0;
}

template <bool TEX_SKY>
__device__ __forceinline__ void gbuffer_store(const SceneView &S, const GBufferArgs &G, DRay &r, size_t i) {
    finish_uv(S, r);
    if (G.hit) {
        rt_hit h;
        h.t = r.t; h.obj = r.obj; h.u = r.u; h.v = r.v;
        G.hit[i] = h;
    }
    if (!G.normal && !G.albedo) return;
    rt_gnormal n;
    rt_galbedo a;
    if (r.obj < 0) {
        const f3 c = sky_color<TEX_SKY>(S, r.D);
        n.nx = 0.0f; n.ny = 0.0f; n.nz = 0.0f; n.material = -1;
        a.r = c.x; a.g = c.y; a.b = c.z; a.kind = -1;
    } else {
        const f3 I = r.O + r.t * r.D;
        float4 s0 = S.shade[2 * r.obj], s1 = S.shade[2 * r.obj + 1];
        asm volatile("" : "+v"(s0.x), "+v"(s0.y), "+v"(s0.z), "+v"(s0.w), "+v"(s1.x), "+v"(s1.y), "+v"(s1.z), "+v"(s1.w));
        const int mi = __float_as_int(s0.w);
        const float4 *mp = reinterpret_cast<const float4 *>(S.mats + mi);
        float4 q[4] = {mp[0], mp[1], mp[2], kExt ? mp[3] : make_float4(0, 0, 0, 0)};
        asm volatile("" : "+v"(q[0].x), "+v"(q[0].y), "+v"(q[0].z), "+v"(q[0].w), "+v"(q[1].x), "+v"(q[1].y), "+v"(q[1].z),
                          "+v"(q[1].w), "+v"(q[2].x), "+v"(q[2].y), "+v"(q[2].z), "+v"(q[2].w));
        if constexpr (kExt) asm volatile("" : "+v"(q[3].x), "+v"(q[3].y));
        DevMaterial m;
        __builtin_memcpy(&m, q, sizeof(m));
        f3 N = prim_normal(S, s0, s1, I);
        if (dot(N, r.D) > 0) N = -N;
        const f3 c = mat_color(S, m, r, I);
        n.nx = N.x; n.ny = N.y; n.nz = N.z; n.material = mi;
        a.r = c.x; a.g = c.y; a.b = c.z; a.kind = m.kind;
    }
    if (G.normal) G.normal[i] = n;
    if (G.albedo) G.albedo[i] = a;
}
__device__ __forceinline__ void gbuffer_store_ray(const GBufferArgs &G, const DRay &r, size_t i) {
// ... 756 lines not shown
    return v.maxd == 1 ? RT_SKY_OF(v.tex, k_render_work, 1) : RT_SKY_OF(v.tex, k_render_work, 32);
}
static const void *trace_kernel(const FrameVariant &v) {
    switch (v.mode * 64 + v.maxd) {
    case M_PATH * 64 + 1: return RT_SKY_OF(v.tex, k_trace, M_PATH, 1);
    case M_PATH * 64 + 4: return RT_SKY_OF(v.tex, k_trace, M_PATH, 4);
    case M_PATH * 64 + 10: return RT_SKY_OF(v.tex, k_trace, M_PATH, 10);
    case M_PATH * 64 + 32: return RT_SKY_OF(v.tex, k_trace, M_PATH, 32);
    case M_WHITTED * 64 + 1: return RT_SKY_OF(v.tex, k_trace, M_WHITTED, 1);
    }
    return nullptr;
}
static const void *pt_level_kernel(bool level0, bool tex) {
    return level0 ? RT_SKY(tex, k_pt_level0) : RT_SKY(tex, k_pt_level);
}
static const void *pt_lanes_kernel(bool quad, bool tex) {
    return quad ? (tex ? (const void *)k_pt_lanes<true, true> : (const void *)k_pt_lanes<false, true>)
                : (tex ? (const void *)k_pt_lanes<true, false> : (const void *)k_pt_lanes<false, false>);
}
static const void *gbuffer_kernel(const GBufferVariant &v) {
    return v.pixels ? RT_SKY(v.tex, k_gbuffer_pixels) : RT_SKY(v.tex, k_gbuffer);
}
#undef RT_SKY
#undef RT_SKY_OF

static void launch_work(const SceneView &S, const FrameArgs &F, const FrameLaunch &L, uint32_t *tile_work, uint32_t *pixel_work) {
    const size_t cnt = kWorkCounterBytes;
    const int wd = 2u * L.lds_bytes + cnt <= kLdsLaunchMax ? 1 : 0;
    const size_t lds = (wd ? 2u : 1u) * L.lds_bytes + cnt;
    launch_kernel<SceneView, FrameArgs, uint32_t *, uint32_t *, int>(work_kernel(L.v), L.grid, lds, L.stream, S, F, tile_work,
                                                                     pixel_work, wd);
}
static void launch_frame(const SceneView &S, const FrameArgs &F, const FrameLaunch &L) {
    launch_kernel<SceneView, FrameArgs>(frame_kernel(L.v), L.grid, L.lds_bytes, L.stream, S, F);
}
static int resident_blocks(const void *fn, size_t lds) {
    static std::mutex mu;
    static std::map<std::tuple<int, const void *, size_t>, int> cache;
    int dev = 0;
    (void)hipGetDevice(&dev);
    std::lock_guard<std::mutex> g(mu);
    const auto key = std::make_tuple(dev, fn, lds);
    auto it = cache.find(key);
    if (it != cache.end()) return it->second;
    int b = 0;
    if (hipOccupancyMaxActiveBlocksPerMultiprocessor(&b, fn, 256, lds) != hipSuccess || b <= 0) b = 2;
    cache.emplace(key, b);
    return b;
}
static int launch_pt_level(const SceneView &S, const FrameArgs &F, const PathArgs &P, bool tex, size_t lds, uint32_t num_cus,
                           hipStream_t st) {
    const int pc = resident_blocks(pt_level_kernel(false, tex), lds);
    const uint32_t need = (P.npaths + 255u) / 256u;
    const uint32_t grid = P.level == 0 ? need : std::min(need, (uint32_t)pc * num_cus);
    launch_kernel<SceneView, FrameArgs, PathArgs>(pt_level_kernel(P.level == 0, tex), dim3(grid), lds, st, S, F, P);
    return pc * (int)num_cus * 256;
}
static void launch_pt_lanes(const SceneView &S, const FrameArgs &F, const PathArgs &P, bool tex, size_t lds, uint32_t num_cus,
                            hipStream_t st) {
    const void *fn = pt_lanes_kernel(S.quad_lanes && S.quads, tex);
    const uint32_t grid = std::min((P.npaths + 255u) / 256u, (uint32_t)resident_blocks(fn, lds) * num_cus);
    launch_kernel<SceneView, FrameArgs, PathArgs>(fn, dim3(grid), lds, st, S, F, P);
}
static void launch_pt_finish(const FrameArgs &F, const PathArgs &P, bool last, hipStream_t st) {
    hipLaunchKernelGGL(k_pt_finish, dim3((F.ntiles_local * 64u + 255u) / 256u), dim3(256), 0, st, F, P, last ? 1 : 0);
}
static void launch_trace(const SceneView &S, const TraceArgs &A, const FrameVariant &v, size_t lds, hipStream_t st) {
    launch_kernel<SceneView, TraceArgs>(trace_kernel(v), dim3((A.n + 255u) / 256u), lds, st, S, A);
}
static void launch_intersect(const SceneView &S, const rt_ray *rays, rt_hit *hits, uint32_t n, size_t lds, hipStream_t st) {
    hipLaunchKernelGGL(k_intersect, dim3((n + 255) / 256), dim3(256), lds, st, S, rays, hits, n);
}
static void launch_occluded(const SceneView &S, const rt_ray *rays, uint8_t *out, uint32_t n, size_t lds, hipStream_t st) {
    hipLaunchKernelGGL(k_occluded, dim3((n + 255) / 256), dim3(256), lds, st, S, rays, out, n);
}
static void launch_intersect_packet(const SceneView &S, const rt_ray *rays, rt_hit *hits, uint32_t n, hipStream_t st) {
    hipLaunchKernelGGL(k_intersect_packet, dim3((n + 255) / 256), dim3(256), 0, st, S, rays, hits, n);
}
static void launch_gbuffer(const SceneView &S, const FrameArgs &F, const GBufferArgs &G, const GBufferVariant &v, size_t lds,
                           hipStream_t st) {
    const uint32_t grid = v.pixels ? (G.n + 255u) / 256u : (G.ntiles + 3u) / 4u;
    launch_kernel<SceneView, FrameArgs, GBufferArgs>(gbuffer_kernel(v), dim3(grid), lds, st, S, F, G);
}
const Launchers &launchers() {
    static const Launchers table = {launch_frame,    launch_work,     launch_intersect, launch_occluded, launch_intersect_packet,
                                    launch_pt_level, launch_pt_lanes, launch_pt_finish, launch_trace,    launch_gbuffer};
    return table;
}
#if RT_EXT == 0
void launch_heat(const SceneView &S, const FrameArgs &F, size_t lds, hipStream_t st) {
    hipLaunchKernelGGL(k_render_heat, dim3((F.ntiles_local + 3u) / 4u), dim3(256), lds, st, S, F);
}
void launch_visualize(const SceneView &S, const rt_ray *rays, uint32_t *counts, uint32_t n, size_t lds, hipStream_t st) {
    hipLaunchKernelGGL(k_bvh_visualize, dim3((n + 255) / 256), dim3(256), lds, st, S, rays, counts, n);
}
#endif

}


#if RT_EXT == 0
__global__ __launch_bounds__(256) void k_assemble(const uint32_t *__restrict__ gathered, uint32_t cap, uint32_t nshards,
                                                  const uint32_t *__restrict__ where, uint32_t tiles_x, uint32_t ntiles,
                                                  uint32_t W, uint32_t H, uint32_t first, uint32_t *__restrict__ out) {
    const uint32_t wave = blockIdx.x * 4u + (threadIdx.x >> 6), lane = threadIdx.x & 63u;
    const uint32_t groups_x = (tiles_x + 7u) / 8u;
    const uint32_t trow = wave / groups_x, tcol = (wave % groups_x) * 8u + (lane & 7u);
    const uint32_t tiles_y = (ntiles + tiles_x - 1u) / tiles_x;
    if (trow >= tiles_y || tcol >= tiles_x) return;
    const uint32_t tile = trow * tiles_x + tcol, row = lane >> 3;
    const uint32_t y = trow * 8u + row, x = tcol * 8u;
    if (y >= H) return;
    const uint32_t w = where ? where[tile] : 0u;
    const uint32_t shard = where ? (w >> 24) : tile % nshards, local = where ? (w & 0xffffffu) : tile / nshards;
    if (shard < first) return;
    const uint32_t *src = gathered + (size_t)(shard - first) * cap + local * 64u + row * 8u;
    uint32_t *dst = out + (size_t)y * W + x;
    if (x + 8u <= W && ((size_t)y * W + x) % 4u == 0u) {
        const uint4 a = reinterpret_cast<const uint4 *>(src)[0], b = reinterpret_cast<const uint4 *>(src)[1];
        reinterpret_cast<uint4 *>(dst)[0] = a;
        reinterpret_cast<uint4 *>(dst)[1] = b;
    } else {
        for (uint32_t i = 0; i < 8u && x + i < W; ++i) dst[i] = src[i];
    }
}


void launch_assemble(const uint32_t *gathered, uint32_t cap, uint32_t nshards, const uint32_t *where, uint32_t tiles_x,
                     uint32_t ntiles, uint32_t W, uint32_t H, uint32_t *out, hipStream_t st, uint32_t first) {
    const uint32_t waves = ((tiles_x + 7u) / 8u) * ((ntiles + tiles_x - 1u) / tiles_x);
    hipLaunchKernelGGL(k_assemble, dim3((waves + 3u) / 4u), dim3(256), 0, st, gathered, cap, nshards, where, tiles_x,
                       ntiles, W, H, first, out);
}
#endif

}

#if defined(RT_FRAME_PHASES) && !RT_EXT
extern "C" __attribute__((visibility("default"))) int rt_debug_frame_phases(unsigned long long *out, size_t n) {
    if (hipDeviceSynchronize() != hipSuccess) return -1;
    return hipMemcpyFromSymbol(out, HIP_SYMBOL(rt::kcore::rt_frame_phase_buf), n * sizeof(unsigned long long)) == hipSuccess ? 0 : -1;
}
extern "C" __attribute__((visibility("default"))) int rt_debug_frame_phases_clear() {
    void *p = nullptr;
    if (hipDeviceSynchronize() != hipSuccess || hipGetSymbolAddress(&p, HIP_SYMBOL(rt::kcore::rt_frame_phase_buf)) != hipSuccess) return -1;
    return hipMemset(p, 0, sizeof(unsigned long long) * 8u * rt::kcore::kFramePhaseWaves) == hipSuccess ? 0 : -1;
}
#endif
```

advancedgraphicsraytracer_amd/csrc/rt_scene.h:

```cpp
#pragma once
#include <hip/hip_runtime.h>

#include "rt_internal.h"
#include "rt_refit.h"

struct rt_scene {
    int device = 0;
    rt::SceneView view{};
    rt::Bvh bvh;
    uint32_t num_prims = 0;
    uint32_t num_materials = 0;
    uint32_t stack_depth = 0;
    int frame_waves = 0;
    uint32_t num_cus = 256;
    bool has_cubes = false;
    bool quads = false;
    bool quad_lanes = false;
    void *d_quads = nullptr;
    bool walk_fits = true;
    bool nested = true;
    int walk = RT_WALK_LANE;
    bool ext = false;
    bool ext_fixed = false;
    bool pt_lanes = true;
    bool pt_dynamic = true;
    bool pt_wavefront = true;
    uint32_t pt_drain_level = 64;
    double pt_drain_rounds = 0.25;
    uint32_t pt_drain_small = 4;
    double pt_small_rounds = 16.0;
    double pt_small_drain_rounds = 0.125;
    bool tile_order = true;
    uint32_t split_units = 40000;
    bool xcd_order = false;
    uint32_t split_parts = 2;
    int32_t heavy_split = -1;
    uint64_t pt_mem_bytes = 12288ull << 20;
    bool pt_pipeline = true;
    uint32_t pt_slots = 0;
    uint32_t ps_buffers = 0;
    int32_t ps_pipeline = -1;
    uint32_t ps_depth = 2;
    float tune_delay_ms = 100.0f;
    void *d_nodes = nullptr, *d_prims = nullptr, *d_shade = nullptr, *d_mats = nullptr, *d_sky = nullptr;
    void *d_xprims = nullptr, *d_tex = nullptr;
    void *d_scratch = nullptr;
    void *d_cost = nullptr;
    size_t scratch_bytes = 0;
    hipStream_t stream = nullptr;
    rt::RefitState refit;
};

namespace rt {

inline int after_updates(const rt_scene *s, hipStream_t st) {
    if (!s->refit.async.issued) return RT_OK;
    HIP_TRY(hipStreamWaitEvent(st, s->refit.async.done, 0));
    return RT_OK;
}

void scene_tree_fields(rt_scene *s, uint32_t root_word, bool nested, bool bounds_finite);
int fold_updates(rt_scene *s);

}
```

advancedgraphicsraytracer_amd/csrc/rt_scene_edit.hip:

```cpp
#include <hip/hip_runtime.h>

#include <string>
#include <vector>

#include "rt_scene.h"
#include "rt_splice.h"

using namespace rt;

int rt::fold_updates(rt_scene *s) {
    if (!s->refit.async.issued) return RT_OK;
    HIP_TRY(hipSetDevice(s->device));
    uint64_t applied = 0;
    const int rc = drain_updates(s->refit, &applied);
    if (rc != RT_OK) return rc;
    if (applied) {
        s->view.bounds_finite = s->refit.boxes_finite ? 1 : 0;
        if (s->refit.boxes_finite) s->nested = true;
    }
    return RT_OK;
}

namespace {

template <class Body>
int edit_call(const char *name, const char *suffix, Body body) {
    Rebuilt t;
    try {
        return body(std::string(name) + suffix, t);
    } catch (const std::exception &e) {
        free_rebuilt(t);
        return fail(RT_ERR_INVALID, std::string(name) + suffix + ": " + e.what());
    }
}
int enter(rt_scene *s, bool fold = true) {
    if (fold)
        if (int rc = fold_updates(s); rc != RT_OK) return rc;
    HIP_TRY(hipSetDevice(s->device));
    return RT_OK;
}

struct Staged { const char *a = nullptr, *b = nullptr; };
int stage(rt_scene *s, const void *a, size_t abytes, const void *b, size_t bbytes, Staged &d) {
    d = Staged();
    if (!abytes) return RT_OK;
    if (!b) bbytes = 0;
    HIP_TRY(hipSetDevice(s->device));
    HIP_TRY(hipDeviceSynchronize());
    const size_t off = (abytes + 15u) & ~(size_t)15u;
    const int rc = grow(&s->d_scratch, &s->scratch_bytes, bbytes ? off + bbytes : abytes);
    if (rc != RT_OK) return rc;
    char *base = (char *)s->d_scratch;
    HIP_TRY(hipMemcpyAsync(base, a, abytes, hipMemcpyHostToDevice, s->stream));
    if (bbytes) HIP_TRY(hipMemcpyAsync(base + off, b, bbytes, hipMemcpyHostToDevice, s->stream));
    d.a = base;
    d.b = bbytes ? base + off : nullptr;
    return RT_OK;
}

int refit_supported(const rt_scene *s, const std::string &who) {
    if (s->bvh.indices.size() != s->num_prims)
        return fail(RT_ERR_UNSUPPORTED, who + ": an SBVH scene (leaves share primitives) cannot be refitted");
    if (s->quads) return fail(RT_ERR_UNSUPPORTED, who + ": scene built with two-level node records (RT_PT_QUADS=1)");
    return RT_OK;
}
int rebuild_supported(const rt_scene *s, const std::string &who) {
    const int rc = refit_supported(s, who);
    if (rc != RT_OK) return rc;
    if (!s->refit.boxes_finite) return fail(RT_ERR_UNSUPPORTED, who + ": a primitive's box is NaN or infinite");
    return RT_OK;
}
int not_a_triangle(const std::string &who, uint32_t id) {
    return fail(RT_ERR_INVALID, who + ": primitive " + std::to_string(id) + " is not a triangle");
}
int require_triangles(const rt_scene *s, uint32_t first, uint32_t count, const std::string &who) {
    for (uint32_t id = first; id < first + count; ++id)
        if ((s->refit.pinfo[id] & 0x7f) != RT_TRIANGLE) return not_a_triangle(who, id);
    return RT_OK;
}
SceneRecords records_of(rt_scene *s) {
    return SceneRecords{&s->bvh, s->num_prims, s->d_nodes, s->d_prims, s->d_shade, s->d_xprims, s->view.walk_margin};
}
int settle(rt_scene *s, int rc, bool finite) {
    if (rc != RT_OK) return rc;
    s->view.bounds_finite = finite ? 1 : 0;
    if (finite) s->nested = true;
    return RT_OK;
}


const char *const kUpdateNames[3] = {"rt_scene_update_triangles", "rt_scene_transform_triangles", "rt_scene_update_prims"};
const char *const kRefusals[3] = {
    "a vertex is NaN or infinite",
    "a transformed vertex is NaN or infinite",
    "a record's type or material is not the scene's, or a field, transform or box is NaN or infinite",
};
const char *form_of(bool async) { return async ? "_async" : ""; }

int update_refusals(const rt_scene *s, uint32_t first, uint32_t count, const void *recs, const char *what, bool light_stays,
                    bool scene_kind, const std::string &who, bool *empty) {
    const int k = async_arguments(s != nullptr, s ? s->num_prims : 0u, first, count, recs, light_stays);
    *empty = k == kAsyncEmpty;
    if (k == kAsyncNullScene) return fail(RT_ERR_INVALID, who + ": null scene");
    if (k == kAsyncEmpty) return RT_OK;
    if (k == kAsyncNullRecords) return fail(RT_ERR_INVALID, who + ": null " + what);
    if (scene_kind)
        if (int rc = refit_supported(s, who); rc != RT_OK) return rc;
    if (k == kAsyncRange) return fail(RT_ERR_INVALID, who + ": range outside the primitives");
    if (k == kAsyncLight) return fail(RT_ERR_UNSUPPORTED, who + ": the range holds primitive 0 (the light moves through rt_scene_update_prims)");
    return RT_OK;
}

int update_triangles(rt_scene *s, uint32_t first, uint32_t count, const float *verts_dev, void *stream, bool async, uint64_t *ticket) {
    return edit_call(kUpdateNames[0], form_of(async), [&](const std::string &who, Rebuilt &) -> int {
        bool empty = false;
        int rc = update_refusals(s, first, count, verts_dev, "vertices", false, true, who, &empty);
        if (rc != RT_OK || empty) return rc;
        if ((rc = require_triangles(s, first, count, who)) != RT_OK || (rc = enter(s, !async)) != RT_OK) return rc;
// ... 256 lines not shown
int rt_scene_transform_triangles_async(rt_scene *s, const rt_tri_xform *ranges, uint32_t num_ranges, const float *rest_dev,
                                       void *stream, uint64_t *ticket) {
    return transform_triangles(s, ranges, num_ranges, rest_dev, stream, true, ticket);
}

int rt_scene_update_sync(rt_scene *s, rt_update_status *out) {
    if (!s) return fail(RT_ERR_INVALID, "rt_scene_update_sync: null scene");
    if (int rc = fold_updates(s); rc != RT_OK) return rc;
    AsyncUpdates &U = s->refit.async;
    if (out) *out = rt_update_status{U.submitted, U.applied, U.refused, U.first_refused};
    if (U.first_refused) (void)fail(RT_ERR_INVALID, std::string(kUpdateNames[U.first_kind]) + form_of(true) + ": " + kRefusals[U.first_kind]);
    U.first_refused = 0;
    U.first_kind = -1;
    return RT_OK;
}

int rt_scene_rebuild(rt_scene *s, void *stream) {
    return edit_call("rt_scene_rebuild", "", [&](const std::string &who, Rebuilt &t) -> int {
        if (!s) return fail(RT_ERR_INVALID, who + ": null scene");
        int rc = rebuild_supported(s, who);
        if (rc != RT_OK || (rc = enter(s)) != RT_OK || (rc = rebuild(s->refit, records_of(s), (hipStream_t)stream, t)) != RT_OK) return rc;
        swap_in_tree(s, t);
        return RT_OK;
    });
}
int rt_scene_rebuild_stats(const rt_scene *s, uint32_t out[4]) {
    if (!s || !out) return fail(RT_ERR_INVALID, "rt_scene_rebuild_stats: null argument");
    for (int k = 0; k < 4; ++k) out[k] = s->refit.rebuild_stats[k];
    return RT_OK;
}

int rt_scene_splice_triangles(rt_scene *s, uint32_t first, uint32_t remove, const rt_prim *prims_dev, uint32_t insert,
                              void *stream) {
    return edit_call("rt_scene_splice_triangles", "", [&](const std::string &who, Rebuilt &t) -> int {
        bool empty = false;
        int rc = splice_arguments(s, first, remove, prims_dev, insert, who, &empty);
        if (rc != RT_OK || empty || (rc = enter(s)) != RT_OK) return rc;
        const uint32_t n = s->num_prims - remove + insert;
        RefitState &R = s->refit;
        std::vector<uint8_t> pinfo;
        pinfo.reserve(n);
        pinfo.insert(pinfo.end(), R.pinfo.begin(), R.pinfo.begin() + first);
        pinfo.insert(pinfo.end(), insert, (uint8_t)RT_TRIANGLE);
        pinfo.insert(pinfo.end(), R.pinfo.begin() + first + remove, R.pinfo.end());
        std::vector<uint32_t> indices(n, 0u);
        const SpliceEdit e{first, remove, insert, prims_dev, s->num_materials};
        if ((rc = splice(R, records_of(s), e, (hipStream_t)stream, t)) != RT_OK) return rc;
        swap_in_splice(s, t, pinfo, indices);
        return RT_OK;
    });
}
int rt_scene_splice_triangles_host(rt_scene *s, uint32_t first, uint32_t remove, const rt_prim *prims, uint32_t insert) {
    bool empty = false;
    Staged d;
    int rc = splice_arguments(s, first, remove, prims, insert, "rt_scene_splice_triangles_host", &empty);
    if (rc != RT_OK || empty || (rc = stage(s, prims, sizeof(rt_prim) * (size_t)insert, nullptr, 0, d)) != RT_OK) return rc;
    return rt_scene_splice_triangles(s, first, remove, (const rt_prim *)d.a, insert, s->stream);
}

int rt_scene_splice_ranges(rt_scene *s, const rt_tri_edit *edits, uint32_t num_edits, const rt_prim *prims_dev, void *stream) {
    return splice_edits(s, edits, num_edits, prims_dev, nullptr, stream, false);
}
int rt_scene_splice_ranges_host(rt_scene *s, const rt_tri_edit *edits, uint32_t num_edits, const rt_prim *prims) {
    return splice_edits_host(s, edits, num_edits, prims, nullptr, false);
}
int rt_scene_splice_prims(rt_scene *s, const rt_prim_edit *edits, uint32_t num_edits, const rt_prim *prims_dev,
                          const float *transforms_dev, void *stream) {
    return splice_edits(s, edits, num_edits, prims_dev, transforms_dev, stream, true);
}
int rt_scene_splice_prims_host(rt_scene *s, const rt_prim_edit *edits, uint32_t num_edits, const rt_prim *prims,
                               const float *transforms) {
    return splice_edits_host(s, edits, num_edits, prims, transforms, true);
}

int rt_scene_compact_triangles(rt_scene *s, const uint8_t *keep_dev, void *stream) { return compact(s, keep_dev, stream, false); }
int rt_scene_compact_triangles_host(rt_scene *s, const uint8_t *keep) { return compact_host(s, keep, false); }
int rt_scene_compact_prims(rt_scene *s, const uint8_t *keep_dev, void *stream) { return compact(s, keep_dev, stream, true); }
int rt_scene_compact_prims_host(rt_scene *s, const uint8_t *keep) { return compact_host(s, keep, true); }

int rt_scene_set_prim_materials(rt_scene *s, uint32_t first, uint32_t count, const int32_t *materials_dev, void *stream) {
    return edit_call("rt_scene_set_prim_materials", "", [&](const std::string &who, Rebuilt &) -> int {
        bool empty = false;
        int rc = materials_arguments(s, first, count, materials_dev, who, &empty);
        if (rc != RT_OK || empty || (rc = enter(s)) != RT_OK) return rc;
        return set_materials(s->refit, records_of(s), first, count, materials_dev, s->num_materials, (hipStream_t)stream);
    });
}
int rt_scene_set_prim_materials_host(rt_scene *s, uint32_t first, uint32_t count, const int32_t *materials) {
    bool empty = false;
    Staged d;
    int rc = materials_arguments(s, first, count, materials, "rt_scene_set_prim_materials_host", &empty);
    if (rc != RT_OK || empty || (rc = stage(s, materials, sizeof(int32_t) * (size_t)count, nullptr, 0, d)) != RT_OK) return rc;
    return rt_scene_set_prim_materials(s, first, count, (const int32_t *)d.a, s->stream);
}


int rt_scene_prepare_updates(rt_scene *s, void *stream) {
    return edit_call("rt_scene_prepare_updates", "", [&](const std::string &who, Rebuilt &) -> int {
        if (!s) return fail(RT_ERR_INVALID, who + ": null scene");
        int rc = refit_supported(s, who);
        if (rc != RT_OK || (rc = enter(s)) != RT_OK) return rc;
        return prepare_updates(s->refit, records_of(s), (hipStream_t)stream);
    });
}

int rt_scene_update_plan_info(const rt_scene *s, uint32_t out[8]) {
    if (!s || !out) return fail(RT_ERR_INVALID, "rt_scene_update_plan_info: null argument");
    if (int frc = fold_updates(const_cast<rt_scene *>(s)); frc != RT_OK) return frc;
    const RefitState &R = s->refit;
    const PlanInfo none{}, &p = R.refit_ready ? R.plan_info : none;
    out[0] = R.refit_ready ? 1u : 0u;
    out[1] = p.route;
    out[2] = R.refit_ready ? R.plan.ntreelets : 0u;
    out[3] = R.refit_ready && R.plan.has_top ? 1u : 0u;
    out[4] = p.list_len;
    out[5] = p.lvl_len;
    out[6] = p.top_nodes;
    out[7] = p.launches;
    return RT_OK;
}

int rt_scene_copy_update_plan(const rt_scene *s, uint32_t *list, uint32_t *lvl, uint32_t *grp) {
    if (!s) return fail(RT_ERR_INVALID, "rt_scene_copy_update_plan: null scene");
    if (int frc = fold_updates(const_cast<rt_scene *>(s)); frc != RT_OK) return frc;
    const RefitState &R = s->refit;
    if (!R.refit_ready) return fail(RT_ERR_INVALID, "rt_scene_copy_update_plan: no schedule is ready (rt_scene_prepare_updates)");
    HIP_TRY(hipSetDevice(s->device));
    if (list) HIP_TRY(hipMemcpy(list, R.d_list, sizeof(uint32_t) * R.plan_info.list_len, hipMemcpyDeviceToHost));
    if (lvl) HIP_TRY(hipMemcpy(lvl, R.d_lvl, sizeof(uint32_t) * R.plan_info.lvl_len, hipMemcpyDeviceToHost));
    if (grp) HIP_TRY(hipMemcpy(grp, R.d_grp, sizeof(uint32_t) * ((size_t)R.plan.ntreelets + 2), hipMemcpyDeviceToHost));
    return RT_OK;
}

}
```

advancedgraphicsraytracer_amd/csrc/rt_sched.h:

```cpp
#pragma once

#include <algorithm>
#include <cstdint>
#include <vector>

namespace rt {

struct TileGrid {
    uint32_t tiles_x, tiles_y, ntiles;
};
inline TileGrid tile_grid(uint32_t W, uint32_t H) {
    const uint32_t tx = (W + 7) / 8, ty = (H + 7) / 8;
    return {tx, ty, tx * ty};
}
inline uint32_t local_tiles(uint32_t ntiles, uint32_t shard, uint32_t nshards) {
    return shard < ntiles ? (ntiles - shard + nshards - 1) / nshards : 0;
}
inline uint64_t frame_pixels(uint32_t W, uint32_t H, uint32_t ntiles_local, uint32_t shard, uint32_t nshards,
                             const uint32_t *list) {
    uint64_t px = (uint64_t)ntiles_local * 64u;
    if ((W & 7u) || (H & 7u)) {
        const TileGrid g = tile_grid(W, H);
        px = 0;
        auto add = [&](uint32_t t) {
            uint32_t tx = t % g.tiles_x, ty = t / g.tiles_x;
            px += (uint64_t)std::min(8u, W - tx * 8) * std::min(8u, H - ty * 8);
        };
        if (list)
            for (uint32_t i = 0; i < ntiles_local; ++i) add(list[i]);
        else
            for (uint32_t t = shard; t < g.ntiles; t += nshards) add(t);
    }
    return px;
}
inline bool held_tiles(int kind, uint32_t ntiles, uint32_t shard, uint32_t nshards, const std::vector<uint32_t> &list,
                       std::vector<uint32_t> &tiles) {
    tiles.clear();
    switch (kind) {
    case 1:
        for (uint32_t t = 0; t < ntiles; ++t) tiles.push_back(t);
        return true;
    case 2:
        for (uint32_t t = shard; t < ntiles; t += nshards) tiles.push_back(t);
        return true;
    case 3:
        tiles = list;
        return true;
    default:
        return false;
    }
}

inline uint32_t sample_chunks(uint32_t spp, uint32_t ntiles_local, uint32_t split_units, bool eligible) {
    uint32_t nchunks = 1;
    if (eligible && spp > 1 && ntiles_local < split_units)
        while (ntiles_local * nchunks < 2u * split_units && nchunks < spp) {
            uint32_t d = nchunks + 1;
            while (spp % d) ++d;
            nchunks = d;
        }
    return nchunks;
}

inline bool tail_bound(const std::vector<uint32_t> &cost, uint32_t num_cus, uint32_t nchunks) {
    double sum = 0, mx = 0;
    for (uint32_t c : cost) { sum += c; mx = std::max<double>(mx, c); }
    const double slots = (double)num_cus * 4.0 * 7.0;
    return sum > 0 && mx * slots > 2.0 * sum * std::max(1u, nchunks);
}
inline uint32_t split_count(uint32_t n, int32_t heavy_split, bool split_ok) {
    if (!split_ok) return 0;
    return std::min<uint32_t>(n, heavy_split < 0 ? n / 32u : (uint32_t)heavy_split);
}
inline uint32_t part_shift(uint32_t parts) { return parts == 8 ? 3u : parts == 4 ? 4u : 5u; }
inline uint32_t order_units(uint32_t ntiles_local, uint32_t nchunks, bool split, uint32_t order_split, uint32_t order_parts) {
    return ntiles_local * nchunks + (split ? order_split * (order_parts - 1u) : 0u);
}
inline uint64_t order_capacity(uint32_t n) { return 9ull * n; }

struct TileWhere {
    uint32_t tiles_x, shard, nshards;
    const uint32_t *map;
};

inline std::vector<uint32_t> xcd_grouped_order(const TileWhere &F, const std::vector<uint32_t> &entries,
                                               const std::vector<uint32_t> &cost, uint32_t parts) {
    const uint32_t n = (uint32_t)entries.size();
    auto morton = [](uint32_t x, uint32_t y) {
        uint64_t m = 0;
        for (int b = 0; b < 16; ++b) m |= (uint64_t)((x >> b) & 1u) << (2 * b) | (uint64_t)((y >> b) & 1u) << (2 * b + 1);
        return m;
    };
    std::vector<uint32_t> z(n);
    std::vector<uint64_t> code(n);
    std::vector<double> ec(n);
    double total = 0;
    for (uint32_t i = 0; i < n; ++i) {
        const uint32_t e = entries[i], lt = e & 0x0fffffffu;
        const uint32_t tile = F.map ? F.map[lt] : lt * F.nshards + F.shard;
        code[i] = morton(tile % F.tiles_x, tile / F.tiles_x) * 16u + (e >> 28);
        ec[i] = (e >> 31) ? cost[lt] / (double)parts : (double)cost[lt];
        z[i] = i;
        total += ec[i];
    }
    std::stable_sort(z.begin(), z.end(), [&](uint32_t a, uint32_t b) { return code[a] < code[b]; });
    std::vector<std::vector<uint32_t>> region(8);
    std::vector<double> left(8, 0.0);
    double acc = 0;
    for (uint32_t i = 0; i < n; ++i) {
        const uint32_t g = std::min<uint32_t>(7u, (uint32_t)(acc * 8.0 / std::max(total, 1.0)));
        region[g].push_back(z[i]);
        left[g] += ec[z[i]];
        acc += ec[z[i]];
    }
    for (auto &rg : region)
        std::stable_sort(rg.begin(), rg.end(), [&](uint32_t a, uint32_t b) { return ec[a] < ec[b]; });
    std::vector<uint32_t> out;
    out.reserve(n);
    for (uint32_t b = 0; out.size() < n; ++b) {
        for (uint32_t w = 0; w < 4 && out.size() < n; ++w) {
            uint32_t g = b % 8u;
            if (region[g].empty()) {
                int best = -1;
                for (uint32_t h = 0; h < 8; ++h)
                    if (!region[h].empty() && (best < 0 || left[h] > left[best])) best = (int)h;
                g = (uint32_t)best;
            }
            const uint32_t i = region[g].back();
            region[g].pop_back();
            left[g] -= ec[i];
            out.push_back(entries[i]);
        }
    }
    return out;
}

inline std::vector<uint32_t> build_tile_order(const std::vector<uint32_t> &cost, uint32_t k, uint32_t parts, bool xcd,
                                              const TileWhere &where) {
    const uint32_t n = (uint32_t)cost.size();
    std::vector<uint32_t> ord(n);
    for (uint32_t i = 0; i < n; ++i) ord[i] = i;
    std::stable_sort(ord.begin(), ord.end(), [&](uint32_t a, uint32_t b) { return cost[a] > cost[b]; });
    std::vector<uint32_t> ent(ord), sp;
    for (uint32_t i = 0; i < k; ++i)
        for (uint32_t q = 0; q < parts; ++q) sp.push_back(ord[i] | 0x80000000u | (q << 28));
    for (uint32_t i = k; i < n; ++i) sp.push_back(ord[i]);
    if (xcd) {
        ent = xcd_grouped_order(where, ord, cost, parts);
        sp = xcd_grouped_order(where, sp, cost, parts);
    }
    ent.insert(ent.end(), sp.begin(), sp.end());
    return ent;
}

struct PathPlan {
    uint64_t per_path, batch, np, seg_cap, qbytes, cbytes, need;
};
inline PathPlan path_plan(uint32_t spp, uint32_t depth, uint64_t npix, uint64_t budget, uint32_t segs) {
    PathPlan p{};
    p.per_path = 32u + 16u + 8u + (uint64_t)(depth - 1) * 32u;
    p.batch = std::max<uint64_t>(1, budget / (p.per_path * npix));
    p.batch = std::min<uint64_t>(p.batch, spp);
    if (p.batch * npix > 0xffffffffull / 2) p.batch = std::max<uint64_t>(1, (0xffffffffull / 2) / npix);
    p.np = p.batch * npix;
    p.seg_cap = ((p.np / 64u + segs - 1) / segs + 1) * 64u;
    p.qbytes = p.seg_cap * segs * 4u;
    p.cbytes = (uint64_t)(depth + 1) * (2u * segs) * 64u;
    p.need = p.np * (p.per_path - 8u) + 2 * p.qbytes + p.cbytes + 4096u;
    return p;
}
inline uint32_t path_slots(uint32_t forced, uint64_t np, int hw_queues, uint64_t need, double avail) {
    uint32_t k = forced ? forced : (np <= (8400u << 10) && hw_queues >= 8 ? 8u : 4u);
    while (k > 2 && (double)k * need + (8ull << 30) > avail) --k;
    return k;
}

}
```

include/rt_amd.h:

```cpp
#ifndef RT_AMD_H
#define RT_AMD_H
#include <stddef.h>
#include <stdint.h>

#ifdef __cplusplus
extern "C" {
#endif

#define RT_ABI_VERSION 4

enum {
    RT_OK = 0,
    RT_ERR_INVALID = -1,
    RT_ERR_NO_DEVICE = -2,
    RT_ERR_HIP = -3,
    RT_ERR_IO = -4,
    RT_ERR_UNSUPPORTED = -5,
    RT_ERR_COMM = -6
};

enum { RT_SPHERE = 0, RT_PLANE = 1, RT_CUBE = 2, RT_QUAD = 3, RT_TRIANGLE = 4 };
enum { RT_DIFFUSE = 0, RT_MIRROR = 1, RT_DIELECTRIC = 2, RT_CHECKERBOARD = 3, RT_LIGHT = 4, RT_DSMIX = 5,
       RT_TEXTURE = 6 };
enum { RT_MODE_PATH = 0, RT_MODE_WHITTED = 1, RT_MODE_PACKET = 2, RT_MODE_BVH_HEAT = 3 };
// ... 106 lines not shown
                          const float *transforms_dev, void *stream);
int rt_scene_splice_prims_host(rt_scene *s, const rt_prim_edit *edits, uint32_t num_edits, const rt_prim *prims,
                               const float *transforms);
int rt_scene_compact_prims(rt_scene *s, const uint8_t *keep_dev, void *stream);
int rt_scene_compact_prims_host(rt_scene *s, const uint8_t *keep);
int rt_scene_set_prim_materials(rt_scene *s, uint32_t first, uint32_t count, const int32_t *materials_dev, void *stream);
int rt_scene_set_prim_materials_host(rt_scene *s, uint32_t first, uint32_t count, const int32_t *materials);
int rt_scene_bvh_cost(rt_scene *s, rt_bvh_cost *out, void *stream);

int rt_intersect(rt_scene *s, const rt_ray *rays_dev, rt_hit *hits_dev, uint32_t n, void *stream);
int rt_occluded(rt_scene *s, const rt_ray *rays_dev, uint8_t *out_dev, uint32_t n, void *stream);
int rt_intersect_packets(rt_scene *s, const rt_ray *rays_dev, rt_hit *hits_dev, uint32_t n, void *stream);
int rt_intersect_host(rt_scene *s, const rt_ray *rays, rt_hit *hits, uint32_t n);
int rt_occluded_host(rt_scene *s, const rt_ray *rays, uint8_t *out, uint32_t n);
int rt_intersect_packets_host(rt_scene *s, const rt_ray *rays, rt_hit *hits, uint32_t n);
int rt_bvh_visualize(rt_scene *s, const rt_ray *rays_dev, uint32_t *counts_dev, uint32_t n, void *stream);
int rt_bvh_visualize_host(rt_scene *s, const rt_ray *rays, uint32_t *counts, uint32_t n);
int rt_bvh_visualize_nodes(const void *nodes, uint32_t nodes_used, const rt_ray *rays, uint32_t *counts, uint32_t n);

int rt_trace(rt_scene *s, int mode, const rt_ray *rays_dev, uint32_t *seeds_dev, const uint8_t *flags_dev,
             uint32_t depth, float *radiance_dev, rt_hit *hits_dev, uint64_t *ray_counts_dev, uint32_t n, void *stream);
int rt_trace_host(rt_scene *s, int mode, const rt_ray *rays, uint32_t *seeds, const uint8_t *flags, uint32_t depth,
                  float *radiance, rt_hit *hits, uint64_t *ray_counts, uint32_t n);

int rt_camera_default(uint32_t width, uint32_t height, rt_camera *out);
int rt_renderer_create(rt_scene *s, uint32_t width, uint32_t height, rt_renderer **out);
int rt_renderer_destroy(rt_renderer *r);
int rt_render_frame(rt_renderer *r, const rt_camera *cam, const rt_frame_params *p, uint32_t *rgb8_dev, void *stream);
int rt_render_frame_host(rt_renderer *r, const rt_camera *cam, const rt_frame_params *p, uint32_t *rgb8_host);

typedef struct { float nx, ny, nz; int32_t material; } rt_gnormal;
typedef struct { float r, g, b;   int32_t kind;     } rt_galbedo;

typedef struct {
    rt_ray     *ray;
    rt_hit     *hit;
    rt_gnormal *normal;
    rt_galbedo *albedo;
} rt_gbuffer;

int rt_render_gbuffer(rt_renderer *r, const rt_camera *cam, const rt_frame_params *p, uint32_t sample,
                      uint32_t x0, uint32_t y0, uint32_t w, uint32_t h, const rt_gbuffer *out_dev, void *stream);
int rt_render_gbuffer_host(rt_renderer *r, const rt_camera *cam, const rt_frame_params *p, uint32_t sample,
                           uint32_t x0, uint32_t y0, uint32_t w, uint32_t h, const rt_gbuffer *out);
int rt_gbuffer_pixels(rt_renderer *r, const rt_camera *cam, const rt_frame_params *p, uint32_t sample,
                      const uint32_t *pixels_dev, uint32_t n, const rt_gbuffer *out_dev, void *stream);
int rt_gbuffer_pixels_host(rt_renderer *r, const rt_camera *cam, const rt_frame_params *p, uint32_t sample,
                           const uint32_t *pixels, uint32_t n, const rt_gbuffer *out);
int rt_renderer_gbuffer_walk(const rt_renderer *r, int pixels, int *wave_walk, uint32_t *lds_bytes);
int rt_shard_capacity(uint32_t width, uint32_t height, uint32_t num_shards, uint32_t *pixels);
int rt_render_shard(rt_renderer *r, const rt_camera *cam, const rt_frame_params *p, uint32_t shard,
                    uint32_t num_shards, uint32_t *tiles_dev, void *stream);
int rt_assemble_shards(rt_renderer *r, const uint32_t *gathered_dev, uint32_t num_shards, uint32_t *rgb8_dev,
                       void *stream);
int rt_tile_deal(uint32_t width, uint32_t height, const uint32_t *cost, uint32_t num_shards, uint32_t *deal_tiles,
                 uint32_t *deal_off);
int rt_render_shard_tiles(rt_renderer *r, const rt_camera *cam, const rt_frame_params *p, const uint32_t *tiles,
                          uint32_t num_tiles, uint32_t *tiles_dev, void *stream);
int rt_assemble_tiles(rt_renderer *r, const uint32_t *gathered_dev, uint32_t stride_px, const uint32_t *deal_tiles,
                      const uint32_t *deal_off, uint32_t num_shards, uint32_t *rgb8_dev, void *stream);
#define RT_COMM_ID_BYTES 128
typedef struct rt_comm rt_comm;
int rt_comm_unique_id(uint8_t id[RT_COMM_ID_BYTES]);
int rt_comm_create(const uint8_t id[RT_COMM_ID_BYTES], int rank, int world, int device, rt_comm **out);
int rt_comm_wrap(void *nccl_comm, int device, rt_comm **out);
int rt_comm_info(const rt_comm *c, int *rank, int *world);
int rt_comm_destroy(rt_comm *c);
#define RT_MULTI_PIPELINED 1u
#define RT_MULTI_TIMING 2u
#define RT_MULTI_BALANCED 4u
int rt_render_frame_multi(rt_renderer *r, rt_comm *c, const rt_camera *cam, const rt_frame_params *p,
                          uint32_t *rgb8_dev, uint32_t flags, void *stream);
int rt_multi_flush(rt_renderer *r, rt_comm *c, uint32_t *rgb8_dev, void *stream);
int rt_comm_timing(rt_comm *c, double *render_ms, double *gather_ms, uint64_t *frames);
int rt_comm_deal_info(const rt_comm *c, int *balanced, uint32_t *ntiles, uint32_t *tile_list, uint64_t stats[4]);
int rt_comm_deal_hash(const rt_comm *c, uint64_t *hash);

int rt_renderer_counters(rt_renderer *r, rt_counters *out);
int rt_renderer_overlap(const rt_renderer *r, int *state, float ms[4]);
int rt_renderer_overlap_depth(const rt_renderer *r, int *depth, float ms[8]);
int rt_renderer_device_bytes(const rt_renderer *r, uint64_t *bytes, uint32_t *ps_buffers);
int rt_renderer_choices(const rt_renderer *r, int *walk, int *split, float walk_ms[4], float split_ms[4]);
int rt_renderer_tile_costs(const rt_renderer *r, uint32_t *costs, uint32_t n, uint32_t *n_out);
int rt_renderer_tile_work(rt_renderer *r, const rt_camera *cam, const rt_frame_params *p, uint32_t *work, uint32_t n,
                          uint32_t *pixel_work_dev, void *stream);
enum { RT_WALK_CHECK_OFF = 0, RT_WALK_CHECK_COUNT = 1, RT_WALK_CHECK_VERIFY = 2 };
int rt_renderer_set_walk_check(rt_renderer *r, int level);
int rt_renderer_walk_stats(rt_renderer *r, uint64_t out[4]);
int rt_renderer_read_accumulator(rt_renderer *r, float *host_out);
const char *rt_frame_kernel_name(const rt_renderer *r, const rt_frame_params *p);
int rt_renderer_stream(rt_renderer *r, void **stream);
int rt_synchronize(rt_renderer *r);

#ifdef __cplusplus
}
#endif
#endif
```

Before: 36950.

## Classify sky-only tiles via interval BVH test and skip their primary traversal

Adds a per-tile conservative interval-arithmetic test that bounds all camera rays of an 8x8 tile and walks the top BVH levels to prove no geometry box can be entered. Tiles proven sky-only get a flag bit in the order entries and the frame kernel skips primary ray traversal for them, writing the constant sky colour when the sky is not textured. The classification is cached per camera key and geometry sequence, with a quiet-frame hysteresis and cross-stream event waits. Costs are an extra small kernel on recompute, a narrowed tile-index mask, and the risk of incorrect pixels if the bound is not conservative.

```diff
diff --git a/advancedgraphicsraytracer_amd/__init__.py b/advancedgraphicsraytracer_amd/__init__.py
--- a/advancedgraphicsraytracer_amd/__init__.py
+++ b/advancedgraphicsraytracer_amd/__init__.py
@@ -227,6 +227,7 @@
         "rt_renderer_overlap_depth": ([vp, C.POINTER(C.c_int), fp], C.c_int),
         "rt_renderer_device_bytes": ([vp, C.POINTER(C.c_uint64), C.POINTER(C.c_uint32)], C.c_int),
         "rt_renderer_tile_costs": ([vp, C.POINTER(u32), u32, C.POINTER(u32)], C.c_int),
+        "rt_renderer_sky_tiles": ([vp, C.POINTER(u32), u32, C.POINTER(u32)], C.c_int),
         "rt_renderer_tile_work": ([vp, C.POINTER(Camera), C.POINTER(FrameParams), C.POINTER(u32), u32, vp, vp], C.c_int),
         "rt_renderer_choices": ([vp, C.POINTER(C.c_int), C.POINTER(C.c_int), fp, fp], C.c_int),
         "rt_renderer_set_walk_check": ([vp, C.c_int], C.c_int),
@@ -1194,6 +1195,14 @@
             _check(self.L.rt_renderer_tile_costs(self.h, out.ctypes.data_as(C.POINTER(C.c_uint32)), n.value, C.byref(n)))
         return out
 
+    def sky_tiles(self):
+        n = C.c_uint32()
+        _check(self.L.rt_renderer_sky_tiles(self.h, None, 0, C.byref(n)))
+        out = np.zeros(n.value, np.uint32)
+        if n.value:
+            _check(self.L.rt_renderer_sky_tiles(self.h, out.ctypes.data_as(C.POINTER(C.c_uint32)), n.value, C.byref(n)))
+        return out
+
     def tile_work(self, spp=1, depth=None, frame=None, pixels=False, stream=None):
         tx, ty = (self.width + 7) // 8, (self.height + 7) // 8
         work = np.zeros(tx * ty, np.uint32)
diff --git a/advancedgraphicsraytracer_amd/build.py b/advancedgraphicsraytracer_amd/build.py
--- a/advancedgraphicsraytracer_amd/build.py
+++ b/advancedgraphicsraytracer_amd/build.py
@@ -9,7 +9,7 @@
 SOURCES = ["rt_host.cpp", "rt_device.hip", "rt_kern_core.hip", "rt_kern_ext.hip", "rt_multi.cpp", "rt_sbvh.cpp",
            "rt_refit.hip", "rt_build.hip", "rt_splice.hip", "rt_scene_pack.cpp", "rt_cost.hip", "rt_plan.hip", "rt_scene_edit.hip"]
 HEADERS = ["rt_math.h", "rt_internal.h", "rt_libm.h", "rt_dev_types.h", "rt_variants.h", "rt_kernels.inc", "rt_refit.h", "rt_tune.h", "rt_sched.h",
-           "rt_records.h", "rt_update.h", "rt_build.h", "rt_splice.h", "rt_cost.h", "rt_plan.h", "rt_scene.h", os.path.join("..", "..", "include", "rt_amd.h")]
+           "rt_records.h", "rt_update.h", "rt_build.h", "rt_splice.h", "rt_cost.h", "rt_plan.h", "rt_scene.h", "rt_sky_tiles.h", os.path.join("..", "..", "include", "rt_amd.h")]
 
 HIPCC = os.environ.get("HIPCC", "/opt/rocm/bin/hipcc")
 LIBS = ["-lz", "-ldl"]
diff --git a/advancedgraphicsraytracer_amd/csrc/rt_dev_types.h b/advancedgraphicsraytracer_amd/csrc/rt_dev_types.h
--- a/advancedgraphicsraytracer_amd/csrc/rt_dev_types.h
+++ b/advancedgraphicsraytracer_amd/csrc/rt_dev_types.h
@@ -4,6 +4,7 @@
 #include <cstdint>
 
 #include "../../include/rt_amd.h"
+#include "rt_sky_tiles.h"
 #include "rt_variants.h"
 
 namespace rt {
@@ -66,6 +67,7 @@
     int packed_out;
     const uint32_t *order;
     uint32_t part_shift;
+    uint32_t sky_skip;
     uint32_t *tile_cost;
     float4 *acc;
     uint32_t *out;
@@ -134,6 +136,7 @@
     void (*trace)(const SceneView &S, const TraceArgs &A, const FrameVariant &v, size_t lds, hipStream_t st);
     void (*gbuffer)(const SceneView &S, const FrameArgs &F, const GBufferArgs &G, const GBufferVariant &v, size_t lds,
                     hipStream_t st);
+    void (*sky_tiles)(const SceneView &S, const FrameArgs &F, uint32_t *order, uint32_t n, hipStream_t st);
 };
 namespace kext {
 const Launchers &launchers();
diff --git a/advancedgraphicsraytracer_amd/csrc/rt_device.hip b/advancedgraphicsraytracer_amd/csrc/rt_device.hip
--- a/advancedgraphicsraytracer_amd/csrc/rt_device.hip
+++ b/advancedgraphicsraytracer_amd/csrc/rt_device.hip
@@ -69,6 +69,14 @@
     int order_state = 0;
     uint32_t order_split = 0;
     uint32_t order_parts = 2;
+    uint32_t order_entries = 0;
+    bool sky_have = false;
+    bool sky_on = false;
+    uint64_t sky_key = 0, sky_seq = 0;
+    uint64_t sky_geom = 0;
+    uint32_t sky_quiet = 0;
+    hipEvent_t sky_ev = nullptr;
+    uint32_t sky_wait = 0;
     TimedGroups walk_tg, split_tg, ps_tg;
     hipEvent_t tune_ev[4][16] = {};
     float walk_ms[4] = {}, split_ms[4] = {}, ps_ms[8] = {};
@@ -192,6 +200,7 @@
     if (const char *e = std::getenv("RT_PT_SMALL_ROUNDS")) s->pt_small_rounds = std::max(0.0, std::atof(e));
     if (const char *e = std::getenv("RT_PT_SMALL_DRAIN_ROUNDS")) s->pt_small_drain_rounds = std::max(0.0, std::atof(e));
     if (const char *e = std::getenv("RT_TILE_ORDER")) s->tile_order = std::atoi(e) != 0;
+    if (const char *e = std::getenv("RT_SKY_TILES")) s->sky_tiles = std::atoi(e) != 0;
     if (const char *e = std::getenv("RT_SPLIT_UNITS")) s->split_units = (uint32_t)std::max(0, std::atoi(e));
     if (const char *e = std::getenv("RT_FRAME_WAVES")) {
         const int w = std::atoi(e);
@@ -512,6 +521,8 @@
         HIP_TRY(hipMemcpy(d_order, ent.data(), ent.size() * sizeof(uint32_t), hipMemcpyHostToDevice));
         r->order_split = k;
         r->order_parts = parts;
+        r->order_entries = (uint32_t)ent.size();
+        r->sky_have = false;
         r->order_state = 2;
         r->use_split = k > 0 && r->scene->heavy_split > 0;
         r->split_tg.stop();
@@ -531,6 +542,38 @@
         F.nunits = order_units(F.ntiles_local, F.nchunks, split, r->order_split, r->order_parts);
         F.part_shift = part_shift(r->order_parts);
     }
+    return RT_OK;
+}
+
+constexpr uint32_t kSkyQuietFrames = 8;
+int sky_step(rt_renderer *r, FrameArgs &F, const SceneView &view, int mode, uint64_t key, hipStream_t st) {
+    rt_scene *s = r->scene;
+    F.sky_skip = 0;
+    r->sky_on = false;
+    const uint64_t seq = s->geometry_seq;
+    if (seq != r->sky_geom) {
+        r->sky_geom = seq;
+        r->sky_quiet = 0;
+    }
+    const uint32_t quiet = r->sky_quiet;
+    if (r->sky_quiet < kSkyQuietFrames) ++r->sky_quiet;
+    if (!s->sky_tiles || r->order_state != 2 || !F.order || F.depth == 0 || mode == RT_MODE_PACKET ||
+        (view.wave_primary && view.walk_check != RT_WALK_CHECK_OFF))
+        return RT_OK;
+    const bool have = r->sky_have && r->sky_key == key;
+    if (!(have && r->sky_seq == seq)) {
+        if (have && quiet < kSkyQuietFrames) return RT_OK;
+        launchers(s).sky_tiles(s->view, F, r->d_order.as<uint32_t>(), r->order_entries, st);
+        HIP_TRY(hipGetLastError());
+        if (!r->sky_ev) HIP_TRY(hipEventCreateWithFlags(&r->sky_ev, hipEventDisableTiming | hipEventReleaseToDevice));
+        HIP_TRY(hipEventRecord(r->sky_ev, st));
+        r->sky_wait = ~0u;
+        r->sky_have = true;
+        r->sky_key = key;
+        r->sky_seq = seq;
+    }
+    F.sky_skip = 1;
+    r->sky_on = true;
     return RT_OK;
 }
 
@@ -835,6 +878,11 @@
     if (int rc = overlap_step(r, F, L, ps_ok, ps_bytes, st, P); rc != RT_OK) return rc;
     if (L.stream != st)
         if (int rc = after_updates(s, L.stream); rc != RT_OK) return rc;
+    if (int rc = sky_step(r, F, view, mode, P.key, st); rc != RT_OK) return rc;
+    if (F.sky_skip && L.stream != st && (r->sky_wait >> P.lane & 1u)) {
+        HIP_TRY(hipStreamWaitEvent(L.stream, r->sky_ev, 0));
+        r->sky_wait &= ~(1u << P.lane);
+    }
     L.lds_bytes = stack_bytes(s) + walk_bytes(s, view);
     L.v = frame_variant({mode, p->depth, !view.sky_const, s->frame_waves, F.nchunks, F.spp, F.nunits, s->num_cus,
                          P.depth > 0, view.wave_primary, view.walk_check});
@@ -1256,7 +1304,7 @@
         if (e) (void)hipEventDestroy(e);
     for (hipEvent_t e : r->ps_res.fin)
         if (e) (void)hipEventDestroy(e);
-    for (hipEvent_t e : {r->ps_join, r->cost_ev, r->stall_ev})
+    for (hipEvent_t e : {r->ps_join, r->cost_ev, r->stall_ev, r->sky_ev})
         if (e) (void)hipEventDestroy(e);
     (void)hipStreamDestroy(r->stream);
     delete r;
@@ -1502,6 +1550,23 @@
     return RT_OK;
 }
 
+int rt_renderer_sky_tiles(rt_renderer *r, uint32_t *tiles, uint32_t n, uint32_t *n_out) {
+    if (!r || !n_out || (n && !tiles)) return fail(RT_ERR_INVALID, "rt_renderer_sky_tiles: null argument");
+    *n_out = 0;
+    if (!r->sky_on || !r->sky_have || r->order_state != 2 || r->sky_seq != r->scene->geometry_seq) return RT_OK;
+    HIP_TRY(hipSetDevice(r->scene->device));
+    HIP_TRY(hipDeviceSynchronize());
+    std::vector<uint32_t> ent(r->order_n);
+    HIP_TRY(hipMemcpy(ent.data(), r->d_order.as<uint32_t>(), ent.size() * sizeof(uint32_t), hipMemcpyDeviceToHost));
+    std::vector<uint32_t> sky;
+    for (uint32_t e : ent)
+        if (e & kEntrySky) sky.push_back(e & kEntryTileMask);
+    std::sort(sky.begin(), sky.end());
+    *n_out = (uint32_t)sky.size();
+    if (n) std::memcpy(tiles, sky.data(), sizeof(uint32_t) * std::min<size_t>(n, sky.size()));
+    return RT_OK;
+}
+
 int rt_renderer_read_accumulator(rt_renderer *r, float *host) {
     if (!r || !host) return fail(RT_ERR_INVALID, "null argument");
     HIP_TRY(hipSetDevice(r->scene->device));
diff --git a/advancedgraphicsraytracer_amd/csrc/rt_kernels.inc b/advancedgraphicsraytracer_amd/csrc/rt_kernels.inc
--- a/advancedgraphicsraytracer_amd/csrc/rt_kernels.inc
+++ b/advancedgraphicsraytracer_amd/csrc/rt_kernels.inc
@@ -900,7 +900,7 @@
 
 template <int MAXD, bool TEX_SKY, class TR, int CAMWAVE = 0, bool WHOLE = false>
 __device__ f3 trace_path(const SceneView &S, const TR &T, DRay ray, int depth, uint32_t &seed,
-                         uint32_t &nshadow, uint32_t &nbounce, bool lastSpec = true) {
+                         uint32_t &nshadow, uint32_t &nbounce, bool lastSpec = true, bool no_walk = false) {
     f3 lv_mul[MAXD], lv_add[MAXD];
     float lv_c[MAXD];
     bool lv_diff[MAXD];
@@ -908,7 +908,8 @@
     f3 term = mk(0, 0, 0);
     for (int d = depth; d > 0 && levels < MAXD; --d) {
         if (d != depth) ++nbounce;
-        if constexpr (CAMWAVE) {
+        if (TEX_SKY && no_walk && d == depth) {
+        } else if constexpr (CAMWAVE) {
             if (d == depth) closest_hit_primary<CAMWAVE == 2>(S, T, ray);
             else closest_hit(S, T, ray);
         } else {
@@ -1045,7 +1046,7 @@
 
 template <bool TEX_SKY, class TR>
 __device__ f3 trace_whitted(const SceneView &S, const TR &T, DRay ray, int depth, uint32_t &seed,
-                            uint32_t &nshadow, uint32_t &nbounce) {
+                            uint32_t &nshadow, uint32_t &nbounce, bool no_walk = false) {
     WFrame st[kWHITTED_MAX];
     int sp = 0;
     bool primary = true;
@@ -1053,8 +1054,8 @@
         f3 ret = mk(0, 0, 0);
         if (depth - sp > 0) {
             if (!primary) ++nbounce;
+            if (!(TEX_SKY && no_walk && primary)) closest_hit(S, T, ray);
             primary = false;
-            closest_hit(S, T, ray);
             if (ray.obj == -1) {
                 ret = sky_color<TEX_SKY>(S, ray.D);
             } else {
@@ -1187,7 +1188,9 @@
     frame_phase(0);
     const uint32_t slot = F.nchunks <= 1 ? unit : unit / F.nchunks;
     const uint32_t entry = F.order ? F.order[slot] : slot;
-    const uint32_t local_tile = entry & 0x0fffffffu;
+    const uint32_t local_tile = entry & kEntryTileMask;
+    constexpr bool kSkySkip = !DRY && !WALKCHECK && MODE != M_PACKET;
+    const bool sky_tile = kSkySkip && __builtin_amdgcn_readfirstlane(entry & kEntrySky) != 0u && F.sky_skip != 0u;
     const bool part_tile = (entry >> 31) != 0u;
     const uint32_t chunk = F.nchunks <= 1 ? 0u : unit % F.nchunks;
     const uint64_t t_start = F.tile_cost ? __builtin_amdgcn_s_memtime() : 0;
@@ -1221,20 +1224,28 @@
             if (on) sum = sum + shade_packet<MAXD, TEX_SKY>(S, T, ray, (int)F.depth, seed, nshadow, nbounce);
         }
     } else if (ONE && on) {
-        uint32_t seed = init_seed(px + F.W * F.H * (s_begin + F.spp * F.frame));
-        DRay ray = primary_ray(F, x, y, seed);
-        frame_phase(1);
-        sum = trace_path<MAXD, TEX_SKY, TR, kCamWave, true>(S, T, ray, (int)F.depth, seed, nshadow, nbounce);
+        if (!TEX_SKY && sky_tile) {
+            sum = sky_color<TEX_SKY>(S, mk(0, 0, 0));
+        } else {
+            uint32_t seed = init_seed(px + F.W * F.H * (s_begin + F.spp * F.frame));
+            DRay ray = primary_ray(F, x, y, seed);
+            frame_phase(1);
+            sum = trace_path<MAXD, TEX_SKY, TR, kCamWave, true>(S, T, ray, (int)F.depth, seed, nshadow, nbounce, true, sky_tile);
+        }
         if (F.samples) {
             F.samples[((size_t)s_begin * F.ntiles_local + local_tile) * 64u + lane] = make_float4(sum.x, sum.y, sum.z, 0.0f);
         }
     } else if (on) {
         for (uint32_t s = s_begin; s < s_end; ++s) {
-            uint32_t seed = init_seed(px + F.W * F.H * (s + F.spp * F.frame));
-            DRay ray = primary_ray(F, x, y, seed);
             f3 v;
-            if constexpr (MODE == M_WHITTED) v = trace_whitted<TEX_SKY>(S, T, ray, (int)F.depth, seed, nshadow, nbounce);
-            else v = trace_path<MAXD, TEX_SKY, TR, kCamWave>(S, T, ray, (int)F.depth, seed, nshadow, nbounce);
+            if (!TEX_SKY && sky_tile) {
+                v = sky_color<TEX_SKY>(S, mk(0, 0, 0));
+            } else {
+                uint32_t seed = init_seed(px + F.W * F.H * (s + F.spp * F.frame));
+                DRay ray = primary_ray(F, x, y, seed);
+                if constexpr (MODE == M_WHITTED) v = trace_whitted<TEX_SKY>(S, T, ray, (int)F.depth, seed, nshadow, nbounce, sky_tile);
+                else v = trace_path<MAXD, TEX_SKY, TR, kCamWave>(S, T, ray, (int)F.depth, seed, nshadow, nbounce, true, sky_tile);
+            }
             if (F.samples) F.samples[((size_t)s * F.ntiles_local + local_tile) * 64u + lane] = make_float4(v.x, v.y, v.z, 0.0f);
             else sum = sum + v;
         }
@@ -1321,6 +1332,21 @@
             q[1] = make_uint4(work[1024], work[1280], 0u, 0u);
         }
     }
+}
+
+__global__ __launch_bounds__(256) void k_sky_tiles(SceneView S, FrameArgs F, uint32_t *__restrict__ order, uint32_t n) {
+    const uint32_t i = blockIdx.x * 256u + threadIdx.x;
+    if (i >= n) return;
+    const uint32_t entry = order[i] & ~kEntrySky;
+    const uint32_t local_tile = entry & kEntryTileMask;
+    if (local_tile >= F.ntiles_local) return;
+    SkyCamera c;
+    for (int k = 0; k < 3; ++k) {
+        c.pos[k] = F.cam_pos[k]; c.tl[k] = F.cam_tl[k]; c.tr[k] = F.cam_tr[k]; c.bl[k] = F.cam_bl[k];
+    }
+    c.lens = F.lens; c.rw = F.rw; c.rh = F.rh;
+    const bool sky = tile_sees_only_sky(reinterpret_cast<const float *>(S.nodes), S.root_word, c, F.tiles_x, global_tile(F, local_tile));
+    order[i] = sky ? entry | kEntrySky : entry;
 }
 
 __global__ __launch_bounds__(256) void k_intersect(SceneView S, const rt_ray *__restrict__ rays, rt_hit *__restrict__ hits,
@@ -2243,9 +2269,13 @@
     const uint32_t grid = v.pixels ? (G.n + 255u) / 256u : (G.ntiles + 3u) / 4u;
     launch_kernel<SceneView, FrameArgs, GBufferArgs>(gbuffer_kernel(v), dim3(grid), lds, st, S, F, G);
 }
+static void launch_sky_tiles(const SceneView &S, const FrameArgs &F, uint32_t *order, uint32_t n, hipStream_t st) {
+    hipLaunchKernelGGL(k_sky_tiles, dim3((n + 255u) / 256u), dim3(256), 0, st, S, F, order, n);
+}
 const Launchers &launchers() {
     static const Launchers table = {launch_frame,    launch_work,     launch_intersect, launch_occluded, launch_intersect_packet,
-                                    launch_pt_level, launch_pt_lanes, launch_pt_finish, launch_trace,    launch_gbuffer};
+                                    launch_pt_level, launch_pt_lanes, launch_pt_finish, launch_trace,    launch_gbuffer,
+                                    launch_sky_tiles};
     return table;
 }
 #if RT_EXT == 0
diff --git a/advancedgraphicsraytracer_amd/csrc/rt_scene.h b/advancedgraphicsraytracer_amd/csrc/rt_scene.h
--- a/advancedgraphicsraytracer_amd/csrc/rt_scene.h
+++ b/advancedgraphicsraytracer_amd/csrc/rt_scene.h
@@ -31,6 +31,8 @@
     double pt_small_rounds = 16.0;
     double pt_small_drain_rounds = 0.125;
     bool tile_order = true;
+    bool sky_tiles = true;
+    uint64_t geometry_seq = 0;
     uint32_t split_units = 40000;
     bool xcd_order = false;
     uint32_t split_parts = 2;
diff --git a/advancedgraphicsraytracer_amd/csrc/rt_scene_edit.hip b/advancedgraphicsraytracer_amd/csrc/rt_scene_edit.hip
--- a/advancedgraphicsraytracer_amd/csrc/rt_scene_edit.hip
+++ b/advancedgraphicsraytracer_amd/csrc/rt_scene_edit.hip
@@ -33,7 +33,8 @@
         return fail(RT_ERR_INVALID, std::string(name) + suffix + ": " + e.what());
     }
 }
-int enter(rt_scene *s, bool fold = true) {
+int enter(rt_scene *s, bool fold = true, bool geometry = true) {
+    if (geometry) ++s->geometry_seq;
     if (fold)
         if (int rc = fold_updates(s); rc != RT_OK) return rc;
     HIP_TRY(hipSetDevice(s->device));
@@ -456,7 +457,7 @@
     return edit_call("rt_scene_set_prim_materials", "", [&](const std::string &who, Rebuilt &) -> int {
         bool empty = false;
         int rc = materials_arguments(s, first, count, materials_dev, who, &empty);
-        if (rc != RT_OK || empty || (rc = enter(s)) != RT_OK) return rc;
+        if (rc != RT_OK || empty || (rc = enter(s, true, false)) != RT_OK) return rc;
         return set_materials(s->refit, records_of(s), first, count, materials_dev, s->num_materials, (hipStream_t)stream);
     });
 }
@@ -473,7 +474,7 @@
     return edit_call("rt_scene_prepare_updates", "", [&](const std::string &who, Rebuilt &) -> int {
         if (!s) return fail(RT_ERR_INVALID, who + ": null scene");
         int rc = refit_supported(s, who);
-        if (rc != RT_OK || (rc = enter(s)) != RT_OK) return rc;
+        if (rc != RT_OK || (rc = enter(s, true, false)) != RT_OK) return rc;
         return prepare_updates(s->refit, records_of(s), (hipStream_t)stream);
     });
 }
diff --git a/advancedgraphicsraytracer_amd/csrc/rt_sched.h b/advancedgraphicsraytracer_amd/csrc/rt_sched.h
--- a/advancedgraphicsraytracer_amd/csrc/rt_sched.h
+++ b/advancedgraphicsraytracer_amd/csrc/rt_sched.h
@@ -3,6 +3,8 @@
 #include <algorithm>
 #include <cstdint>
 #include <vector>
+
+#include "rt_sky_tiles.h"
 
 namespace rt {
 
@@ -96,7 +98,7 @@
     std::vector<double> ec(n);
     double total = 0;
     for (uint32_t i = 0; i < n; ++i) {
-        const uint32_t e = entries[i], lt = e & 0x0fffffffu;
+        const uint32_t e = entries[i], lt = e & kEntryTileMask;
         const uint32_t tile = F.map ? F.map[lt] : lt * F.nshards + F.shard;
         code[i] = morton(tile % F.tiles_x, tile / F.tiles_x) * 16u + (e >> 28);
         ec[i] = (e >> 31) ? cost[lt] / (double)parts : (double)cost[lt];
diff --git a/advancedgraphicsraytracer_amd/csrc/rt_sky_tiles.h b/advancedgraphicsraytracer_amd/csrc/rt_sky_tiles.h
--- /dev/null
+++ b/advancedgraphicsraytracer_amd/csrc/rt_sky_tiles.h
@@ -0,0 +1,115 @@
+#pragma once
+#include <stdint.h>
+
+#include <cmath>
+
+#if defined(__HIPCC__) || defined(__CUDACC__)
+#define RT_SKY_HD __host__ __device__ inline
+#else
+#define RT_SKY_HD inline
+#endif
+
+namespace rt {
+
+constexpr uint32_t kEntrySky = 1u << 27;
+constexpr uint32_t kEntryTileMask = kEntrySky - 1u;
+constexpr uint32_t kSkyBudget = 64;
+
+struct Iv { float lo, hi; };
+
+RT_SKY_HD float iv_min(float a, float b) { return (a != a || b != b) ? NAN : (b < a ? b : a); }
+RT_SKY_HD float iv_max(float a, float b) { return (a != a || b != b) ? NAN : (a < b ? b : a); }
+RT_SKY_HD bool iv_nan(Iv a) { return a.lo != a.lo || a.hi != a.hi; }
+RT_SKY_HD bool iv_finite(Iv a) { return std::fabs(a.lo) <= 3.4028234664e38f && std::fabs(a.hi) <= 3.4028234664e38f; }
+RT_SKY_HD bool iv_has_zero(Iv a) { return !(a.lo > 0.0f || a.hi < 0.0f); }
+
+RT_SKY_HD Iv iv(float x) { return Iv{x, x}; }
+RT_SKY_HD Iv iv(float lo, float hi) { return Iv{lo, hi}; }
+RT_SKY_HD Iv iv_add(Iv a, Iv b) { return Iv{a.lo + b.lo, a.hi + b.hi}; }
+RT_SKY_HD Iv iv_sub(Iv a, Iv b) { return Iv{a.lo - b.hi, a.hi - b.lo}; }
+RT_SKY_HD Iv iv_mul(Iv a, Iv b) {
+    const float p0 = a.lo * b.lo, p1 = a.lo * b.hi, p2 = a.hi * b.lo, p3 = a.hi * b.hi;
+    return Iv{iv_min(iv_min(p0, p1), iv_min(p2, p3)), iv_max(iv_max(p0, p1), iv_max(p2, p3))};
+}
+RT_SKY_HD Iv iv_sqr(Iv a) {
+    const float p0 = a.lo * a.lo, p1 = a.hi * a.hi;
+    return Iv{iv_has_zero(a) ? (iv_nan(a) ? NAN : 0.0f) : iv_min(p0, p1), iv_max(p0, p1)};
+}
+RT_SKY_HD Iv iv_rcp(Iv a) { return Iv{1.0f / a.hi, 1.0f / a.lo}; }
+RT_SKY_HD Iv iv_sqrt(Iv a) { return Iv{sqrtf(a.lo), sqrtf(a.hi)}; }
+
+struct SkyCamera {
+    float pos[3], tl[3], tr[3], bl[3];
+    float lens, rw, rh;
+};
+
+RT_SKY_HD bool tile_ray_bounds(const SkyCamera &c, uint32_t tx, uint32_t ty, Iv O[3], Iv rD[3]) {
+    const Iv x = iv((float)(8u * tx), (float)(8u * tx + 7u)), y = iv((float)(8u * ty), (float)(8u * ty + 7u));
+    const Iv rnd = iv(0.0f, 1.0f), sym = iv(-1.0f, 1.0f);
+    const Iv u = iv_add(iv_mul(x, iv(c.rw)), iv_mul(rnd, iv(c.rw)));
+    const Iv v = iv_add(iv_mul(y, iv(c.rh)), iv_mul(rnd, iv(c.rh)));
+    const Iv rdx = iv_mul(iv(c.lens), sym), rdy = iv_mul(iv(c.lens), sym);
+    const Iv off[3] = {iv_mul(u, rdx), iv_mul(v, rdy), iv(0.0f)};
+    Iv d[3];
+    for (int k = 0; k < 3; ++k) {
+        const Iv P = iv_add(iv_add(iv(c.tl[k]), iv_mul(u, iv(c.tr[k] - c.tl[k]))), iv_mul(v, iv(c.bl[k] - c.tl[k])));
+        O[k] = iv_add(iv(c.pos[k]), off[k]);
+        d[k] = iv_sub(iv_sub(P, iv(c.pos[k])), off[k]);
+    }
+    const Iv len2 = iv_add(iv_add(iv_sqr(d[0]), iv_sqr(d[1])), iv_sqr(d[2]));
+    if (!(len2.lo > 0.0f) || iv_nan(len2)) return false;
+    const Iv inv = iv_rcp(iv_sqrt(len2));
+    for (int k = 0; k < 3; ++k) {
+        const Iv D = iv_mul(d[k], inv);
+        if (iv_has_zero(D)) return false;
+        rD[k] = iv_rcp(D);
+        if (!iv_finite(rD[k]) || !iv_finite(O[k])) return false;
+    }
+    return true;
+}
+
+RT_SKY_HD bool box_may_be_entered(const Iv O[3], const Iv rD[3], const float mn[3], const float mx[3]) {
+    float tmn_lo = 0.0f, tmx_hi = 0.0f;
+    for (int k = 0; k < 3; ++k) {
+        const Iv t1 = iv_mul(iv_sub(iv(mn[k]), O[k]), rD[k]), t2 = iv_mul(iv_sub(iv(mx[k]), O[k]), rD[k]);
+        const float lo = iv_min(t1.lo, t2.lo), hi = iv_max(t1.hi, t2.hi);
+        tmn_lo = k == 0 ? lo : iv_max(tmn_lo, lo);
+        tmx_hi = k == 0 ? hi : iv_min(tmx_hi, hi);
+    }
+    if (tmn_lo != tmn_lo || tmx_hi != tmx_hi) return true;
+    return !(tmx_hi < tmn_lo || tmx_hi <= 0.0f);
+}
+
+RT_SKY_HD uint32_t sky_word(float f) {
+    uint32_t u;
+    __builtin_memcpy(&u, &f, sizeof(u));
+    return u;
+}
+
+RT_SKY_HD bool rays_see_only_sky(const float *nodes, uint32_t root_word, const Iv O[3], const Iv rD[3]) {
+    if (root_word & 0xffu) return false;
+    uint32_t stack[kSkyBudget];
+    uint32_t sp = 0, tests = 0;
+    uint32_t word = root_word;
+    for (;;) {
+        const float *q = nodes + (size_t)(word >> 8) * 8u;
+        for (int c = 0; c < 2; ++c, q += 8) {
+            if (++tests > kSkyBudget) return false;
+            const float mn[3] = {q[0], q[1], q[2]}, mx[3] = {q[3], q[4], q[5]};
+            if (!box_may_be_entered(O, rD, mn, mx)) continue;
+            const uint32_t w = sky_word(q[6]);
+            if (w & 0xffu) return false;
+            stack[sp++] = w;
+        }
+        if (sp == 0) return true;
+        word = stack[--sp];
+    }
+}
+
+RT_SKY_HD bool tile_sees_only_sky(const float *nodes, uint32_t root_word, const SkyCamera &c, uint32_t tiles_x, uint32_t tile) {
+    Iv O[3], rD[3];
+    if (!tile_ray_bounds(c, tile % tiles_x, tile / tiles_x, O, rD)) return false;
+    return rays_see_only_sky(nodes, root_word, O, rD);
+}
+
+}
diff --git a/include/rt_amd.h b/include/rt_amd.h
--- a/include/rt_amd.h
+++ b/include/rt_amd.h
@@ -212,6 +212,7 @@
 int rt_renderer_device_bytes(const rt_renderer *r, uint64_t *bytes, uint32_t *ps_buffers);
 int rt_renderer_choices(const rt_renderer *r, int *walk, int *split, float walk_ms[4], float split_ms[4]);
 int rt_renderer_tile_costs(const rt_renderer *r, uint32_t *costs, uint32_t n, uint32_t *n_out);
+int rt_renderer_sky_tiles(rt_renderer *r, uint32_t *tiles, uint32_t n, uint32_t *n_out);
 int rt_renderer_tile_work(rt_renderer *r, const rt_camera *cam, const rt_frame_params *p, uint32_t *work, uint32_t n,
                           uint32_t *pixel_work_dev, void *stream);
 enum { RT_WALK_CHECK_OFF = 0, RT_WALK_CHECK_COUNT = 1, RT_WALK_CHECK_VERIFY = 2 };
```

Measured after the change: 37280 (median of 6 runs). Within noise of the previous version (+0.9%).
